# shaohua-pan/RobustCap

Measured on AMD Instinct MI355X. Metric: body-frames/sec (sig_mp fwd + FK) at batch 256, higher is better.
Workload: dtype f32; 1 GPU; synthetic 60 fps, 6 IMU + 33 keypoints, batch 256 x 1448 frames per GPU (256 bodies in total, weak scaling), confidence schedule 'mixed', seeded random weights (63.4 M params); batch_per_gpu=256, bodies_total=256, frames=1448, conf=mixed, parallelism=dp1 (sequence sharding)

## Files before the change

### include/robustcap_hip.h

```cpp
#ifndef ROBUSTCAP_HIP_H
#define ROBUSTCAP_HIP_H

#include <stdint.h>

#ifdef __cplusplus
extern "C" {
#endif

typedef struct rc_ctx rc_ctx;

typedef enum {
    RC_OK = 0,
    RC_ERR_INVALID = -1,
    RC_ERR_HIP = -2,
    RC_ERR_STATE = -3,
    RC_ERR_UNKNOWN_KEY = -4
} rc_status;

typedef struct {
    double conf_lo, conf_hi;
    float contact_threshold;
    float distance_threshold;
    float height_threshold;
    double tran_filter_num;
    int32_t use_flat_floor;
    int32_t use_vision_updater;
    int32_t use_imu_updater;
    int32_t live;
    int32_t update_vision_freq;
    int32_t use_reproj_opt;
    float smooth;
    int32_t reserved;
} rc_params;

#define RC_FLAG_FIRST_FRAME 1u

int rc_create(int32_t batch, int32_t live_at_construction, rc_ctx** out);
int rc_destroy(rc_ctx* ctx);
const char* rc_last_error(const rc_ctx* ctx);
int rc_default_params(int32_t live_at_construction, rc_params* out);
int rc_get_params(const rc_ctx* ctx, rc_params* out);
int rc_set_params(rc_ctx* ctx, const rc_params* p);

int rc_load_weight(rc_ctx* ctx, const char* key, const float* host, int64_t numel);
int rc_finalize_weights(rc_ctx* ctx);

int rc_set_body(rc_ctx* ctx, const int32_t* parent, const float* J, const float* w33, const float* v33);

int rc_set_gravity(rc_ctx* ctx, const float* gravity_host);

int rc_reset(rc_ctx* ctx, const uint8_t* row_mask, void* stream);

int rc_step(rc_ctx* ctx, const float* j2dc, const float* accc, const float* oric, const float* first_tran,
            uint32_t flags, float* pose_out, float* tran_out, void* stream);

int rc_sequence(rc_ctx* ctx, int32_t T, const float* j2dc, int64_t rs_j2d, const float* accc, int64_t rs_acc,
                const float* oric, int64_t rs_ori, const float* first_tran, uint32_t flags, float* pose_out,
                int64_t rs_pose, float* tran_out, int64_t rs_tran, void* stream);

int rc_sequence_rows(rc_ctx* ctx, int32_t T, const int32_t* len_host, const float* j2dc, int64_t rs_j2d, const float* accc,
                     int64_t rs_acc, const float* oric, int64_t rs_ori, const float* first_tran, uint32_t flags, float* pose_out,
                     int64_t rs_pose, float* tran_out, int64_t rs_tran, void* stream);
int rc_get_sequence_row_frames(rc_ctx* ctx, int64_t* body_frames);

int rc_set_gemm_mode(rc_ctx* ctx, int32_t mode);
int rc_get_gemm_mode(const rc_ctx* ctx);
int rc_default_gemm_mode(int32_t total_rows);

int rc_set_sequence_mode(rc_ctx* ctx, int32_t mode, int32_t min_frames);
int rc_get_sequence_stats(rc_ctx* ctx, int64_t* wave_frames, int64_t* stepped_frames, int64_t* ticks);
int rc_get_launch_stats(rc_ctx* ctx, int64_t* lds_launches, int64_t* other_wide_launches);
int rc_get_launch_stats_w32(rc_ctx* ctx, int64_t* w32_launches);
int rc_set_resident(rc_ctx* ctx, int32_t enable, int32_t workgroups);
int rc_get_resident_stats(rc_ctx* ctx, int64_t* segments, int64_t* aborts);
int rc_plan_sequence(const int8_t* codes, int32_t B, int32_t T, const int32_t* pend, uint32_t flags, int32_t use_vision_updater,
                     uint8_t* mode_out);
int rc_plan_wave(const int8_t* codes, int32_t B, int32_t T, int32_t t0, const int32_t* first_reach, const int32_t* pend,
                 int32_t use_imu_updater, int32_t use_vision_updater, int32_t* frame_at, int64_t frame_at_cap,
                 int32_t* n_ticks, int32_t* n_prep, int32_t* counts, double* est_us);
int rc_plan_wave_rows(const int8_t* codes, int32_t B, int32_t T, int32_t t0, const int32_t* len, const int32_t* first_reach,
                      const int32_t* pend, int32_t use_imu_updater, int32_t use_vision_updater, int32_t* frame_at, int64_t frame_at_cap,
                      int32_t* n_ticks, int32_t* n_prep, int32_t* counts, double* est_us);

int rc_live_begin(rc_ctx* ctx);
int rc_live_step(rc_ctx* ctx, const float* j2dc_host, const float* accc_host, const float* oric_host,
                 const float* first_tran_host, uint32_t flags, float* pose_host, float* tran_host);
int rc_live_end(rc_ctx* ctx);
int rc_get_live_stats(rc_ctx* ctx, int64_t* lean_frames, int64_t* full_frames);
int rc_get_live_prestep(rc_ctx* ctx, int64_t* presteps, int32_t* available);
int rc_get_live_replayed(rc_ctx* ctx, int64_t* frames);
int rc_get_live_spin(rc_ctx* ctx, int64_t* taken, int64_t* lost);
int rc_get_live_profile(rc_ctx* ctx, double* avg_us4);
int rc_get_live_last_profile(rc_ctx* ctx, double* us6);
int rc_get_live_backend(rc_ctx* ctx, int32_t* lean_captured, int32_t* aql, char* note, int32_t note_len);

int rc_r6d_to_rotmat(const float* r6d, float* R, int64_t n, void* stream);
int rc_axis_angle_to_rotmat(const float* aa, float* R, int64_t n, void* stream);
int rc_rotmat_to_axis_angle(const float* R, float* aa, int64_t n, void* stream);
int rc_rotmat_to_r6d(const float* R, float* r6d, int64_t n, void* stream);
int rc_angle_between(const float* R1, const float* R2, float* out, int64_t n, void* stream);
int rc_lerp(const float* a, const float* b, double t, float* out, int64_t n, void* stream);
int rc_normalize_rows(const float* x, float* out, float* norm, int64_t rows, int32_t width, void* stream);
int rc_bbox_normalise(const float* kp, float* out, int64_t n, void* stream);
int rc_conf_mean(const float* j2dc, int64_t n, double lo, double hi, float* mean, int8_t* code, void* stream);
int rc_shape_body(rc_ctx* ctx, const float* v_template, const float* shapedirs, const float* J_regressor, const float* beta,
                  int32_t V, float* verts_out, float* joints_out);
int rc_fk_r(rc_ctx* ctx, const float* Rlocal, float* Rglobal, int64_t n, void* stream);
int rc_bone_to_joint(rc_ctx* ctx, const float* bone, float* joint, int64_t n, void* stream);
int rc_joint_to_bone(rc_ctx* ctx, const float* joint, float* bone, int64_t n, void* stream);
int rc_zero_pose(rc_ctx* ctx, float* joint, float* vert, void* stream);
int rc_ik_r(rc_ctx* ctx, const float* Rglobal, float* Rlocal, int64_t n, void* stream);
int rc_fk_bone(rc_ctx* ctx, const float* Rglobal, float* joints, int64_t n, void* stream);
int rc_body_fk(rc_ctx* ctx, const float* pose, const float* tran, float* grot, float* joint, float* j33,
               int64_t n, void* stream);
int rc_lstm_step(rc_ctx* ctx, const char* net, const float* x, const uint8_t* row_mask, float* y, void* stream);
#define RC_SUBNET_SCRATCH_BYTES (256ll << 20)
int rc_subnet_forward(rc_ctx* ctx, const char* net, int32_t n, const int32_t* lengths_host, const float* x, float* y,
                      const float* init_h, const float* init_c, float* final_h, float* final_c, void* stream);
int rc_subnet_forward_tape(rc_ctx* ctx, const char* net, int32_t n, const int32_t* lengths_host, const float* x, float* y,
                           const float* init_h, const float* init_c, float* final_h, float* final_c, float* acts, float* tape,
                           void* stream);
int rc_subnet_tape_floats(rc_ctx* ctx, const char* net, int32_t n, const int32_t* lengths_host, int64_t* floats);
int rc_subnet_backward(rc_ctx* ctx, const char* net, int32_t n, const int32_t* lengths_host, const float* tape, const float* d_h1,
                       const float* d_final_h, const float* d_final_c, float* d_gates, float* d_a, float* d_init_h, float* d_init_c,
                       void* stream);
int rc_dropout_apply(rc_ctx* ctx, const float* src, float* dst, int64_t rows, int32_t cols, int32_t site, float p, uint64_t seed,
                     uint32_t call, void* stream);
int rc_subnet_forward_train(rc_ctx* ctx, const char* net, int32_t n, const int32_t* lengths_host, const float* x, float* y,
                            const float* init_h, const float* init_c, float* final_h, float* final_c, float* acts, float* tape, float p,
                            uint64_t seed, uint32_t call, void* stream);
int rc_subnet_backward_train(rc_ctx* ctx, const char* net, int32_t n, const int32_t* lengths_host, const float* tape, const float* d_h1,
                             const float* d_final_h, const float* d_final_c, float* d_gates, float* d_a, float* d_init_h,
                             float* d_init_c, float p, uint64_t seed, uint32_t call, void* stream);
int rc_update_subnet_weights(rc_ctx* ctx, const char* net, const void* const* tensors_dev, int32_t count, void* stream);
int rc_subnet_optim_step(rc_ctx* ctx, const char* net, const void* const* params_dev, const void* const* grads_dev,
                         const void* const* exp_avg_dev, const void* const* exp_avg_sq_dev, int32_t count, double lr, double beta1,
                         double beta2, double eps, double weight_decay, double bias_correction1, double bias_correction2, double max_norm,
                         float* norm_out_dev, void* stream);
int rc_init_net_forward(rc_ctx* ctx, int32_t n, const float* v, float* out, void* stream);
int rc_get_subnet_stats(rc_ctx* ctx, int64_t* calls, int64_t* frames, int64_t* chunks, int64_t* scratch_bytes);
int rc_set_mesh(rc_ctx* ctx, const float* v_template_host, const float* weights_host, int32_t V);
int rc_body_mesh(rc_ctx* ctx, const float* pose, const float* tran, float* vert, int64_t n, void* stream);
int rc_set_regressor(rc_ctx* ctx, const float* j_regressor_host, int32_t n_rows, int32_t n_used);
int rc_mesh_metrics(rc_ctx* ctx, const float* pose, const float* gt_pose, int64_t n, float* per_frame, double* mean_host,
                    void* stream);
int rc_synth_imu(rc_ctx* ctx, const float* pose, const float* tran, const int32_t* vertex_ids_host,
                 const int32_t* joint_ids_host, int64_t T, int32_t smooth_n, float* imu_ori, float* imu_acc, float* joint3d,
                 float* vert6, void* stream);
int rc_syn_acc(const float* v, int64_t T, int64_t width, int32_t smooth_n, float* acc, void* stream);
int rc_procrustes_error(const float* S1, const float* S2, int64_t n, int32_t n_points, float* err, void* stream);
int rc_position_error(const float* p, const float* t, int64_t n, float* dist, double* mean_host, void* stream);
int rc_set_ignored_landmarks(rc_ctx* ctx, const int32_t* ids_host, int32_t n);
int rc_reproj_residual(rc_ctx* ctx, const float* pose, const float* tran, const float* kp, const float* K,
                       float sigma, float* loss, int64_t T, void* stream);


int rc_smplify_set_prior(rc_ctx* ctx, const float* means_host, const float* precisions_host, const float* nll_weights_host);

int rc_smplify_loss_grad(rc_ctx* ctx, const float* x, const float* kp, const float* ref3d, const float* imu_aa,
                         const float* K_host, int64_t T, double* loss_host, float* grad, void* stream);

int rc_smplify_set_ref3d(rc_ctx* ctx, const float* ref3d);

typedef struct rc_smplify_info {
    int32_t status;
    int32_t n_iter, n_eval;
    int32_t reserved;
    double first_loss, final_loss;
    double host_ms, device_ms;
} rc_smplify_info;

int rc_smplify_run(rc_ctx* ctx, const float* pose, const float* tran, const float* kp, const float* imu_ori,
                   const float* K_host, int64_t T, float lr, int32_t max_iter, float loss_threshold, float* pose_out,
                   float* tran_out, uint8_t* update_host, rc_smplify_info* info, void* stream);

int rc_smplify_run_batch(rc_ctx* ctx, int32_t n_rows, const int64_t* T_rows, const float* const* pose, const float* const* tran,
                         const float* const* kp, const float* const* imu_ori, const float* K_host, float lr, int32_t max_iter,
                         float loss_threshold, float* const* pose_out, float* const* tran_out, uint8_t* const* update_host,
                         rc_smplify_info* infos, void* stream);

typedef double (*rc_objective_fn)(void* user, const double* x, double* grad, int64_t n);
int rc_lbfgs_minimize(rc_objective_fn objective, void* user, int64_t n, double* x, double lr, int32_t max_iter,
                      int32_t max_eval, int32_t history_size, double tolerance_grad, double tolerance_change,
                      int32_t* n_iter_out, int32_t* n_eval_out, double* losses_out, int64_t cap);

int rc_camera_inputs(const float* kp_pix, const float* imu_acc_w, const float* imu_ori_w, const float* K_host,
                     const float* Tcw_host, float* j2dc, float* accc, float* oric, float* gravity_out_host, int64_t n,
                     void* stream);

int rc_camera_inputs_rows(const float* kp_norm, const float* imu_acc_w, const float* imu_ori_w, const int32_t* seq_of_row,
                          const int32_t* len, const float* K_host, const float* Tcw_host, float image_w, float image_h,
                          int32_t n_rows, int32_t Tmax, float* j2dc, float* accc, float* oric, float* gravity_out_host,
                          void* cam_scratch, void* stream);

int rc_get_state(rc_ctx* ctx, const char* net, float* h_host, float* c_host, void* stream);
int rc_get_fusion_state(rc_ctx* ctx, int32_t* out_host, void* stream);

int rc_get_trace(rc_ctx* ctx, int32_t* trace_host, void* stream);

int rc_gemm_timing(rc_ctx* ctx, int32_t enable);
int rc_gemm_timing_read(rc_ctx* ctx, double* total_ms, int64_t* launches);
int rc_gemm_timing_busy(rc_ctx* ctx, double* busy_ms);

#ifdef __cplusplus
}
#endif
#endif
```

### robustcap_amd/_lib.py

```python
import ctypes as C
import os

_HERE = os.path.dirname(os.path.abspath(__file__))
LIB_PATH = os.environ.get("RC_LIB_PATH") or os.path.join(_HERE, "csrc", "librobustcap_hip.so")
HEADER_PATH = os.path.join(os.path.dirname(_HERE), "include", "robustcap_hip.h")

RC_FLAG_FIRST_FRAME = 1


class RcParams(C.Structure):
    _fields_ = [("conf_lo", C.c_double), ("conf_hi", C.c_double),
                ("contact_threshold", C.c_float), ("distance_threshold", C.c_float),
                ("height_threshold", C.c_float), ("tran_filter_num", C.c_double),
                ("use_flat_floor", C.c_int32), ("use_vision_updater", C.c_int32),
                ("use_imu_updater", C.c_int32), ("live", C.c_int32),
                ("update_vision_freq", C.c_int32), ("use_reproj_opt", C.c_int32), ("smooth", C.c_float),
                ("reserved", C.c_int32)]


class RcSmplifyInfo(C.Structure):
    _fields_ = [("status", C.c_int32), ("n_iter", C.c_int32), ("n_eval", C.c_int32), ("reserved", C.c_int32),
                ("first_loss", C.c_double), ("final_loss", C.c_double), ("host_ms", C.c_double), ("device_ms", C.c_double)]


OBJECTIVE_FN = C.CFUNCTYPE(C.c_double, C.c_void_p, C.POINTER(C.c_double), C.POINTER(C.c_double), C.c_int64)


class RobustcapLibraryError(RuntimeError):
    pass


_P, _I32, _I64, _U32, _F = C.c_void_p, C.c_int32, C.c_int64, C.c_uint32, C.c_float
SIGNATURES = {
    "rc_create": (_I32, [_I32, _I32, C.POINTER(_P)]),
    "rc_destroy": (_I32, [_P]),
    "rc_last_error": (C.c_char_p, [_P]),
    "rc_default_params": (_I32, [_I32, C.POINTER(RcParams)]),
    "rc_get_params": (_I32, [_P, C.POINTER(RcParams)]),
    "rc_set_params": (_I32, [_P, C.POINTER(RcParams)]),
    "rc_load_weight": (_I32, [_P, C.c_char_p, _P, _I64]),
    "rc_finalize_weights": (_I32, [_P]),
    "rc_set_body": (_I32, [_P, _P, _P, _P, _P]),
    "rc_set_gravity": (_I32, [_P, _P]),
    "rc_reset": (_I32, [_P, _P, _P]),
    "rc_step": (_I32, [_P, _P, _P, _P, _P, _U32, _P, _P, _P]),
    "rc_sequence": (_I32, [_P, _I32, _P, _I64, _P, _I64, _P, _I64, _P, _U32, _P, _I64, _P, _I64, _P]),
    "rc_sequence_rows": (_I32, [_P, _I32, _P, _P, _I64, _P, _I64, _P, _I64, _P, _U32, _P, _I64, _P, _I64, _P]),
    "rc_get_sequence_row_frames": (_I32, [_P, C.POINTER(_I64)]),
    "rc_set_gemm_mode": (_I32, [_P, _I32]),
    "rc_get_gemm_mode": (_I32, [_P]),
    "rc_default_gemm_mode": (_I32, [_I32]),
    "rc_set_sequence_mode": (_I32, [_P, _I32, _I32]),
    "rc_get_sequence_stats": (_I32, [_P, C.POINTER(_I64), C.POINTER(_I64), C.POINTER(_I64)]),
    "rc_get_launch_stats": (_I32, [_P, C.POINTER(_I64), C.POINTER(_I64)]),
    "rc_get_launch_stats_w32": (_I32, [_P, C.POINTER(_I64)]),
    "rc_set_resident": (_I32, [_P, _I32, _I32]),
    "rc_get_resident_stats": (_I32, [_P, C.POINTER(_I64), C.POINTER(_I64)]),
    "rc_plan_sequence": (_I32, [_P, _I32, _I32, _P, _U32, _I32, _P]),
    "rc_plan_wave": (_I32, [_P, _I32, _I32, _I32, _P, _P, _I32, _I32, _P, _I64, C.POINTER(_I32), C.POINTER(_I32), _P, _P]),
    "rc_plan_wave_rows": (_I32, [_P, _I32, _I32, _I32, _P, _P, _P, _I32, _I32, _P, _I64, C.POINTER(_I32), C.POINTER(_I32), _P, _P]),
    "rc_live_begin": (_I32, [_P]),
    "rc_live_step": (_I32, [_P, _P, _P, _P, _P, _U32, _P, _P]),
    "rc_live_end": (_I32, [_P]),
    "rc_get_live_stats": (_I32, [_P, _P, _P]),
    "rc_get_live_prestep": (_I32, [_P, _P, _P]),
    "rc_get_live_replayed": (_I32, [_P, _P]),
    "rc_get_live_spin": (_I32, [_P, _P, _P]),
    "rc_get_live_profile": (_I32, [_P, _P]),
    "rc_get_live_last_profile": (_I32, [_P, _P]),
    "rc_get_live_backend": (_I32, [_P, _P, _P, _P, _I32]),
    "rc_get_fusion_state": (_I32, [_P, _P, _P]),
    "rc_r6d_to_rotmat": (_I32, [_P, _P, _I64, _P]),
    "rc_axis_angle_to_rotmat": (_I32, [_P, _P, _I64, _P]),
    "rc_rotmat_to_axis_angle": (_I32, [_P, _P, _I64, _P]),
    "rc_rotmat_to_r6d": (_I32, [_P, _P, _I64, _P]),
    "rc_angle_between": (_I32, [_P, _P, _P, _I64, _P]),
    "rc_lerp": (_I32, [_P, _P, C.c_double, _P, _I64, _P]),
    "rc_normalize_rows": (_I32, [_P, _P, _P, _I64, _I32, _P]),
    "rc_bbox_normalise": (_I32, [_P, _P, _I64, _P]),
    "rc_conf_mean": (_I32, [_P, _I64, C.c_double, C.c_double, _P, _P, _P]),
    "rc_shape_body": (_I32, [_P, _P, _P, _P, _P, _I32, _P, _P]),
    "rc_fk_r": (_I32, [_P, _P, _P, _I64, _P]),
    "rc_bone_to_joint": (_I32, [_P, _P, _P, _I64, _P]),
    "rc_joint_to_bone": (_I32, [_P, _P, _P, _I64, _P]),
    "rc_zero_pose": (_I32, [_P, _P, _P, _P]),
    "rc_ik_r": (_I32, [_P, _P, _P, _I64, _P]),
    "rc_fk_bone": (_I32, [_P, _P, _P, _I64, _P]),
    "rc_body_fk": (_I32, [_P, _P, _P, _P, _P, _P, _I64, _P]),
    "rc_set_mesh": (_I32, [_P, _P, _P, _I32]),
    "rc_body_mesh": (_I32, [_P, _P, _P, _P, _I64, _P]),
    "rc_set_regressor": (_I32, [_P, _P, _I32, _I32]),
    "rc_mesh_metrics": (_I32, [_P, _P, _P, _I64, _P, C.POINTER(C.c_double), _P]),
    "rc_synth_imu": (_I32, [_P, _P, _P, _P, _P, _I64, _I32, _P, _P, _P, _P, _P]),
    "rc_syn_acc": (_I32, [_P, _I64, _I64, _I32, _P, _P]),
    "rc_procrustes_error": (_I32, [_P, _P, _I64, _I32, _P, _P]),
    "rc_position_error": (_I32, [_P, _P, _I64, _P, C.POINTER(C.c_double), _P]),
    "rc_lstm_step": (_I32, [_P, C.c_char_p, _P, _P, _P, _P]),
    "rc_subnet_forward": (_I32, [_P, C.c_char_p, _I32, _P, _P, _P, _P, _P, _P, _P, _P]),
    "rc_subnet_forward_tape": (_I32, [_P, C.c_char_p, _I32, _P, _P, _P, _P, _P, _P, _P, _P, _P, _P]),
    "rc_subnet_tape_floats": (_I32, [_P, C.c_char_p, _I32, _P, C.POINTER(_I64)]),
    "rc_subnet_backward": (_I32, [_P, C.c_char_p, _I32, _P, _P, _P, _P, _P, _P, _P, _P, _P, _P]),
    "rc_dropout_apply": (_I32, [_P, _P, _P, _I64, _I32, _I32, _F, C.c_uint64, _U32, _P]),
    "rc_subnet_forward_train": (_I32, [_P, C.c_char_p, _I32, _P, _P, _P, _P, _P, _P, _P, _P, _P, _F, C.c_uint64, _U32, _P]),
    "rc_subnet_backward_train": (_I32, [_P, C.c_char_p, _I32, _P, _P, _P, _P, _P, _P, _P, _P, _P, _F, C.c_uint64, _U32, _P]),
    "rc_update_subnet_weights": (_I32, [_P, C.c_char_p, _P, _I32, _P]),
    "rc_subnet_optim_step": (_I32, [_P, C.c_char_p, _P, _P, _P, _P, _I32] + [C.c_double] * 8 + [_P, _P]),
    "rc_init_net_forward": (_I32, [_P, _I32, _P, _P, _P]),
    "rc_get_subnet_stats": (_I32, [_P, C.POINTER(_I64), C.POINTER(_I64), C.POINTER(_I64), C.POINTER(_I64)]),
    "rc_set_ignored_landmarks": (_I32, [_P, _P, _I32]),
    "rc_reproj_residual": (_I32, [_P, _P, _P, _P, _P, _F, _P, _I64, _P]),
    "rc_smplify_set_prior": (_I32, [_P, _P, _P, _P]),
    "rc_smplify_set_ref3d": (_I32, [_P, _P]),
    "rc_smplify_loss_grad": (_I32, [_P, _P, _P, _P, _P, _P, _I64, C.POINTER(C.c_double), _P, _P]),
    "rc_smplify_run": (_I32, [_P, _P, _P, _P, _P, _P, _I64, _F, _I32, _F, _P, _P, _P, C.POINTER(RcSmplifyInfo), _P]),
    "rc_smplify_run_batch": (_I32, [_P, _I32, _P, _P, _P, _P, _P, _P, _F, _I32, _F, _P, _P, _P, _P, _P]),
    "rc_lbfgs_minimize": (_I32, [OBJECTIVE_FN, _P, _I64, C.POINTER(C.c_double), C.c_double, _I32, _I32, _I32, C.c_double,
                                 C.c_double, C.POINTER(_I32), C.POINTER(_I32), C.POINTER(C.c_double), _I64]),
    "rc_camera_inputs": (_I32, [_P, _P, _P, _P, _P, _P, _P, _P, _P, _I64, _P]),
    "rc_camera_inputs_rows": (_I32, [_P, _P, _P, _P, _P, _P, _P, _F, _F, _I32, _I32, _P, _P, _P, _P, _P, _P]),
    "rc_get_state": (_I32, [_P, C.c_char_p, _P, _P, _P]),
    "rc_get_trace": (_I32, [_P, _P, _P]),
    "rc_gemm_timing": (_I32, [_P, _I32]),
    "rc_gemm_timing_read": (_I32, [_P, C.POINTER(C.c_double), C.POINTER(_I64)]),
    "rc_gemm_timing_busy": (_I32, [_P, C.POINTER(C.c_double)]),
}

_lib = None


OPTIONAL_IN_AB_BUILDS = frozenset({"rc_get_launch_stats_w32", "rc_set_resident", "rc_get_resident_stats", "rc_get_launch_stats", "rc_get_live_spin", "rc_get_live_replayed", "rc_get_live_profile", "rc_get_live_last_profile",
                                   "rc_get_live_prestep"})


def load():
    global _lib
    if _lib is not None:
        return _lib
    if not os.path.exists(LIB_PATH):
        raise RobustcapLibraryError(
            f"{LIB_PATH} not found: the HIP extension is not built. Run "
            "`python -c \"import __graft_entry__ as g; g.build()\"` at the repo root. There is no CPU fallback.")
    try:
        lib = C.CDLL(LIB_PATH)
    except OSError as e:
        raise RobustcapLibraryError(f"cannot load {LIB_PATH}: {e}") from e
    ab_build = bool(os.environ.get("RC_LIB_PATH"))
    skipped = []
    for name, (res, args) in SIGNATURES.items():
        if ab_build and name in OPTIONAL_IN_AB_BUILDS and not hasattr(lib, name):
            skipped.append(name)
            continue
        try:
            fn = getattr(lib, name)
        except AttributeError as e:
            raise RobustcapLibraryError(f"{LIB_PATH} does not export {name}: the library does not match include/robustcap_hip.h") from e
        fn.restype, fn.argtypes = res, args
    if skipped:
        import warnings
        warnings.warn(f"RC_LIB_PATH={LIB_PATH}: entry points missing in this build (calls to them will fail): {', '.join(skipped)}")
    _lib = lib
    return lib


def check(ctx, rc, what):
    if rc != 0:
        msg = load().rc_last_error(ctx)
        raise RobustcapLibraryError(f"{what} failed ({rc}): {msg.decode() if msg else ''}")


def ptr(t):
    return None if t is None else C.c_void_p(t.data_ptr())


def stream_ptr():
    import torch
    return C.c_void_p(torch.cuda.current_stream().cuda_stream)
```

### robustcap_amd/csrc/rc_api.cpp

```cpp
#include "../../include/robustcap_hip.h"
#include "rc_ctx.h"

#include <algorithm>
#include <cmath>
#include <cstdio>
#include <cstdlib>
#include <cstring>
#include <map>
#include <string>
#include <thread>
#include <vector>

static thread_local std::string g_create_error;

int fail(rc_ctx* ctx, int code, const std::string& msg) {
    if (ctx) ctx->err = msg; else g_create_error = msg;
    return code;
}

namespace {

const int kInit[3][2] = {{69, 512}, {512, 1024}, {1024, 2048}};

template <typename Body>
// ... 385 lines not shown
    if (!ctx) return RC_ERR_INVALID;
    if (!net || !tensors_dev) return fail(ctx, RC_ERR_INVALID, "rc_update_subnet_weights: null argument");
    const int ni = net_index(net);
    if (ni < 0) return fail(ctx, RC_ERR_INVALID, std::string("rc_update_subnet_weights: unknown net ") + net);
    const int want = ni == N2 ? 18 : 12;
    if (count != want) return fail(ctx, RC_ERR_INVALID, "rc_update_subnet_weights: " + std::string(net) + " has " + std::to_string(want) + " tensors");
    for (int i = 0; i < count; ++i)
        if (!tensors_dev[i]) return fail(ctx, RC_ERR_INVALID, "rc_update_subnet_weights: null tensor");
    if (!ctx->have_weights) return fail(ctx, RC_ERR_STATE, "rc_update_subnet_weights: weights not finalized");
    hipStream_t st = (hipStream_t)stream;
    auto T = [&](int i) { return static_cast<const float*>(tensors_dev[i]); };
    live_forget_last_frame(ctx);
    if (int rc = live_discard_ahead(ctx)) return rc;
    HIP_TRY(ctx, hipDeviceSynchronize());
    NetDev& n = ctx->net[ni];
    auto dense = [&](Dense& d, const float* W, const float* b) -> int {
        rc_launch_repack_dense(W, d.N, d.K, d.Np, d.Kp, d.W, d.Ws, st);
        if (d.Wrm) HIP_TRY(ctx, hipMemcpyAsync(d.Wrm, W, (size_t)d.N * d.K * sizeof(float), hipMemcpyDeviceToDevice, st));
        HIP_TRY(ctx, hipMemcpyAsync(d.b, b, (size_t)d.N * sizeof(float), hipMemcpyDeviceToDevice, st));
        return RC_OK;
    };
    for (int l = 0; l < 2; ++l) rc_launch_repack_lstm(T(4 * l), T(4 * l + 1), T(4 * l + 2), T(4 * l + 3), n.H, n.Wl[l], n.Wls[l], n.bl[l], st);
    if (int rc = dense(n.lin1, T(8), T(9))) return rc;
    if (int rc = dense(n.lin2, T(10), T(11))) return rc;
    if (ni == N2)
        for (int q = 0; q < 3; ++q)
            if (int rc = dense(ctx->init[q], T(12 + 2 * q), T(13 + 2 * q))) return rc;
    rc_subnet_retranspose(ctx->subnet.get(), ni, n.Wl, n.H, ctx->weights_epoch, st);
    HIP_TRY(ctx, hipGetLastError());
    HIP_TRY(ctx, hipStreamSynchronize(st));
    return RC_OK;
}

static long long subnet_tensor_numel(int ni, int i) {
    const NetSpec& s = kNets[ni];
    const long long H = s.H;
    if (i < 8) return (i & 3) < 2 ? 4 * H * H : 4 * H;
    if (i < 12) return i == 8 ? H * s.in : i == 9 ? H : i == 10 ? (long long)s.out * H : s.out;
    const int q = (i - 12) / 2;
    return (i & 1) ? kInit[q][1] : (long long)kInit[q][0] * kInit[q][1];
}

int rc_subnet_optim_step(rc_ctx* ctx, const char* net, const void* const* params_dev, const void* const* grads_dev,
                         const void* const* exp_avg_dev, const void* const* exp_avg_sq_dev, int32_t count, double lr, double beta1,
                         double beta2, double eps, double weight_decay, double bias_correction1, double bias_correction2, double max_norm,
                         float* norm_out_dev, void* stream) {
    if (!ctx) return RC_ERR_INVALID;
    const char* what = "rc_subnet_optim_step: ";
    if (!net || !params_dev || !grads_dev || !exp_avg_dev || !exp_avg_sq_dev || !norm_out_dev)
        return fail(ctx, RC_ERR_INVALID, std::string(what) + "null argument");
    const int ni = net_index(net);
    if (ni < 0) return fail(ctx, RC_ERR_INVALID, std::string(what) + "unknown net " + net);
    const int want = ni == N2 ? 18 : 12;
    if (count != want) return fail(ctx, RC_ERR_INVALID, what + std::string(net) + " has " + std::to_string(want) + " tensors");
    for (int i = 0; i < count; ++i)
        if (!params_dev[i] || !exp_avg_dev[i] || !exp_avg_sq_dev[i]) return fail(ctx, RC_ERR_INVALID, std::string(what) + "null parameter or moment tensor");
    if (!(bias_correction1 > 0.0) || !(bias_correction2 > 0.0)) return fail(ctx, RC_ERR_INVALID, std::string(what) + "bias corrections must be positive");
    if (!ctx->have_weights) return fail(ctx, RC_ERR_STATE, std::string(what) + "weights not finalized");
    hipStream_t st = (hipStream_t)stream;
    if (!ctx->optim_partial) {
        long long most = 0;
        for (int j = 0; j < 6; ++j) {
            long long b = 0;
            for (int i = 0; i < (j == N2 ? 18 : 12); ++i) b += (subnet_tensor_numel(j, i) + RC_OPTIM_CHUNK - 1) / RC_OPTIM_CHUNK;
            most = std::max(most, b);
        }
        HIP_TRY(ctx, rc_alloc(ctx->optim_partial, (size_t)most));
    }
    OptimNorm nrm{};
    nrm.count = count;
    int blocks = 0;
    for (int i = 0; i < count; ++i) {
        nrm.g[i] = static_cast<const float*>(grads_dev[i]);
        nrm.n[i] = subnet_tensor_numel(ni, i);
        nrm.block0[i] = blocks;
        if (nrm.g[i]) blocks += (int)((nrm.n[i] + RC_OPTIM_CHUNK - 1) / RC_OPTIM_CHUNK);
    }
    nrm.block0[count] = blocks;
    OptimScalars a{};
    a.step_size = (float)(lr / bias_correction1); a.bc2_sqrt = (float)std::sqrt(bias_correction2);
    a.beta1 = (float)beta1; a.one_m_beta1 = (float)(1.0 - beta1); a.beta2 = (float)beta2; a.one_m_beta2 = (float)(1.0 - beta2);
    a.eps = (float)eps; a.weight_decay = (float)weight_decay;
    auto T = [&](int i) {
        return OptimTensor{static_cast<float*>(const_cast<void*>(params_dev[i])), static_cast<const float*>(grads_dev[i]),
                           static_cast<float*>(const_cast<void*>(exp_avg_dev[i])), static_cast<float*>(const_cast<void*>(exp_avg_sq_dev[i]))};
    };
    for (int i : {0, 1, 4, 5}) {
        const OptimTensor t = T(i);
        if (((uintptr_t)t.p | (uintptr_t)t.g | (uintptr_t)t.m | (uintptr_t)t.v) & 15)
            return fail(ctx, RC_ERR_INVALID, std::string(what) + "the LSTM weight tensors must be 16-byte aligned");
    }
    live_forget_last_frame(ctx);
    const bool live = live_session_open(ctx);
    if (live) {
        if (int rc = live_discard_ahead(ctx)) return rc;
        HIP_TRY(ctx, hipDeviceSynchronize());
    }
    rc_launch_optim_norm(nrm, blocks, ctx->optim_partial.get(), (float)max_norm, norm_out_dev, st);
    NetDev& n = ctx->net[ni];
    auto dense = [&](Dense& d, int i) { rc_launch_optim_dense(T(i), T(i + 1), d.N, d.K, d.Np, d.Kp, d.W, d.Ws, d.Wrm, d.b, a, norm_out_dev, st); };
    for (int l = 0; l < 2; ++l)
        rc_launch_optim_lstm(T(4 * l), T(4 * l + 1), T(4 * l + 2), T(4 * l + 3), n.H, n.Wl[l], n.Wls[l], n.bl[l], a, norm_out_dev, st);
    dense(n.lin1, 8);
    dense(n.lin2, 10);
    if (ni == N2)
        for (int q = 0; q < 3; ++q) dense(ctx->init[q], 12 + 2 * q);
    rc_subnet_retranspose(ctx->subnet.get(), ni, n.Wl, n.H, ctx->weights_epoch, st);
    HIP_TRY(ctx, hipGetLastError());
    if (live) {
        HIP_TRY(ctx, hipStreamSynchronize(st));
        return RC_OK;
    }
    return mark_eager(ctx, st);
}

static int finalize_weights_impl(rc_ctx* ctx) {
    for (int i = 0; i < 6; ++i) {
        const NetSpec& s = kNets[i];
        NetDev& n = ctx->net[i];
        const std::string p = std::string(s.name) + ".";
        const size_t H = s.H;
        auto need = [&](const std::string& r, size_t numel) { return staged(ctx, p + r, numel); };
        const auto *w1 = need("linear1.weight", H * s.in), *b1 = need("linear1.bias", H);
        const auto *w2 = need("linear2.weight", (size_t)s.out * H), *b2 = need("linear2.bias", s.out);
        if (!w1 || !b1 || !w2 || !b2) return fail(ctx, RC_ERR_STATE, "rc_finalize_weights: missing linear weights of " + p);
        if (int rc = make_dense(ctx, n.lin1, *w1, *b1, s.H, s.in)) return rc;
        if (int rc = make_dense(ctx, n.lin2, *w2, *b2, s.out, s.H)) return rc;
        for (int l = 0; l < 2; ++l) {
            const std::string sl = std::to_string(l);
            const auto *wi = need("rnn.weight_ih_l" + sl, 4 * H * H), *wh = need("rnn.weight_hh_l" + sl, 4 * H * H);
            const auto *bi = need("rnn.bias_ih_l" + sl, 4 * H), *bh = need("rnn.bias_hh_l" + sl, 4 * H);
            if (!wi || !wh || !bi || !bh) return fail(ctx, RC_ERR_STATE, "rc_finalize_weights: missing LSTM weights of " + p);
            auto orig = [&](int np) { const int cb = np / 16, u = (np % 16) / 4, g = np % 4; return (size_t)g * H + 4 * cb + u; };
            auto get = [&](int np, int k) -> float {
                const size_t r = orig(np);
                return k < (int)H ? (*wi)[r * H + k] : (*wh)[r * H + (k - H)];
            };
            std::vector<float> bp(4 * H);
            for (size_t np = 0; np < 4 * H; ++np) bp[np] = (*bi)[orig((int)np)] + (*bh)[orig((int)np)];
            if (int rc = upload(ctx, &n.Wl[l], pack_weights(4 * s.H, 2 * s.H, get))) return rc;
            if (int rc = upload16(ctx, &n.Wls[l], pack_weights_split(4 * s.H, 2 * s.H, get))) return rc;
            if (int rc = upload(ctx, &n.bl[l], bp)) return rc;
        }
    }
    for (int q = 0; q < 3; ++q) {
        const std::string p = "rnn2.init_net." + std::to_string(2 * q) + ".";
        const auto *w = staged(ctx, p + "weight", (size_t)kInit[q][0] * kInit[q][1]), *b = staged(ctx, p + "bias", kInit[q][1]);
        if (!w || !b) return fail(ctx, RC_ERR_STATE, "rc_finalize_weights: missing " + p);
        if (int rc = make_dense(ctx, ctx->init[q], *w, *b, kInit[q][1], kInit[q][0])) return rc;
    }
    ctx->have_weights = true;
    const bool aw = ctx->alloc_weights;
    ctx->alloc_weights = false;
    const int rc_pre = seq_prepare(ctx);
    ctx->alloc_weights = aw;
    if (rc_pre) return rc_pre;
    HIP_TRY(ctx, hipDeviceSynchronize());
    std::map<std::string, std::vector<float>>().swap(ctx->staged);
    return RC_OK;
}

int rc_set_body(rc_ctx* ctx, const int32_t* parent, const float* J, const float* w33, const float* v33) {
    if (!ctx || !parent || !J || !w33 || !v33) return RC_ERR_INVALID;
    BodyConst b{};
    for (int i = 0; i < 24; ++i) {
        b.parent[i] = i == 0 ? 0 : parent[i];
        if (i > 0 && (parent[i] < 0 || parent[i] >= i)) return fail(ctx, RC_ERR_INVALID, "rc_set_body: parent[i] must be in [0, i)");
        b.level[i] = i == 0 ? 0 : b.level[parent[i]] + 1;
        if (b.level[i] > 9) return fail(ctx, RC_ERR_INVALID, "rc_set_body: kinematic tree deeper than 9");
        if (i > 0) {
            int& n = b.nchild[parent[i]];
            if (n >= 4) return fail(ctx, RC_ERR_INVALID, "rc_set_body: a joint with more than 4 children");
            b.child[parent[i]][n++] = i;
        }
    }
    for (int i = 0; i < 24; ++i)
        for (int c = 0; c < 3; ++c) {
            b.jroot[c] = J[c];
            b.jrest[i][c] = J[3 * i + c] - J[c];
            b.bone[i][c] = i == 0 ? b.jrest[0][c] : (J[3 * i + c] - J[c]) - (J[3 * parent[i] + c] - J[c]);
        }
    for (int v = 0; v < 33; ++v) {
        b.override_joint[v] = -1;
        for (int c = 0; c < 3; ++c) b.v33[v][c] = v33[3 * v + c] - J[c];
        for (int j = 0; j < 24; ++j) b.w33[v][j] = w33[24 * v + j];
    }
    const int ov[12][2] = {{11, 16}, {12, 17}, {13, 18}, {14, 19}, {15, 20}, {16, 21},
                           {23, 1},  {24, 2},  {25, 4},  {26, 5},  {27, 7},  {28, 8}};
    for (auto& o : ov) b.override_joint[o[0]] = o[1];
    HIP_TRY(ctx, hipMemcpy(ctx->body, &b, sizeof(b), hipMemcpyHostToDevice));
    ctx->have_body = true;
    for (int c = 0; c < 3; ++c) ctx->jroot_h[c] = b.jroot[c];
    ctx->fold_dirty = true;
    return RC_OK;
}

int rc_set_gravity(rc_ctx* ctx, const float* g) {
    if (!ctx || !g) return RC_ERR_INVALID;
    HIP_TRY(ctx, hipMemcpy(ctx->fb.gravity, g, (size_t)ctx->B * 3 * sizeof(float), hipMemcpyHostToDevice));
    return RC_OK;
}

int rc_reset(rc_ctx* ctx, const uint8_t* row_mask, void* stream) {
    if (!ctx) return RC_ERR_INVALID;
    live_forget_last_frame(ctx, true);
    float* h[6]; float* c[6]; int H[6];
    for (int i = 0; i < 6; ++i) { h[i] = ctx->net[i].h; c[i] = ctx->net[i].c; H[i] = ctx->net[i].H; }
    rc_launch_reset(ctx->fb, h, c, H, row_mask, ctx->B, (hipStream_t)stream);
    HIP_TRY(ctx, hipGetLastError());
    return mark_eager(ctx, (hipStream_t)stream);
}

int rc_step(rc_ctx* ctx, const float* j2dc, const float* accc, const float* oric, const float* first_tran, uint32_t flags,
            float* pose_out, float* tran_out, void* stream) {
    if (int rc = check_ready(ctx)) return rc;
    live_forget_last_frame(ctx);
    if (!j2dc || !accc || !oric || !pose_out || !tran_out) return fail(ctx, RC_ERR_INVALID, "rc_step: null buffer");
    FrameIO io{j2dc, accc, oric, first_tran, pose_out, tran_out, 99, 18, 54, 216, 3};
    if (int rc = step_impl(ctx, io, flags, (hipStream_t)stream)) return rc;
    return mark_eager(ctx, (hipStream_t)stream);
}

int rc_r6d_to_rotmat(const float* r6d, float* R, int64_t n, void* stream) {
    if (n == 0) return RC_OK;
    if (!r6d || !R || n < 0) return RC_ERR_INVALID;
    rc_launch_r6d(r6d, R, n, (hipStream_t)stream);
    return hipGetLastError() == hipSuccess ? RC_OK : RC_ERR_HIP;
}
int rc_axis_angle_to_rotmat(const float* aa, float* R, int64_t n, void* stream) {
    if (n == 0) return RC_OK;
    if (!aa || !R || n < 0) return RC_ERR_INVALID;
    rc_launch_aa2R(aa, R, n, (hipStream_t)stream);
    return hipGetLastError() == hipSuccess ? RC_OK : RC_ERR_HIP;
}
int rc_rotmat_to_axis_angle(const float* R, float* aa, int64_t n, void* stream) {
    if (n == 0) return RC_OK;
    if (!aa || !R || n < 0) return RC_ERR_INVALID;
    rc_launch_R2aa(R, aa, n, (hipStream_t)stream);
    return hipGetLastError() == hipSuccess ? RC_OK : RC_ERR_HIP;
}
int rc_rotmat_to_r6d(const float* R, float* r6d, int64_t n, void* stream) {
    if (n == 0) return RC_OK;
    if (!R || !r6d || n < 0) return RC_ERR_INVALID;
    rc_launch_rotmat_to_r6d(R, r6d, n, (hipStream_t)stream);
    return hipGetLastError() == hipSuccess ? RC_OK : RC_ERR_HIP;
}
int rc_angle_between(const float* R1, const float* R2, float* out, int64_t n, void* stream) {
    if (n == 0) return RC_OK;
    if (!R1 || !R2 || !out || n < 0) return RC_ERR_INVALID;
    rc_launch_angle_between(R1, R2, out, n, (hipStream_t)stream);
    return hipGetLastError() == hipSuccess ? RC_OK : RC_ERR_HIP;
}
int rc_lerp(const float* a, const float* b, double t, float* out, int64_t n, void* stream) {
    if (n == 0) return RC_OK;
    if (!a || !b || !out || n < 0) return RC_ERR_INVALID;
    rc_launch_lerp(a, b, (float)(1.0 - t), (float)t, out, n, (hipStream_t)stream);
    return hipGetLastError() == hipSuccess ? RC_OK : RC_ERR_HIP;
}
int rc_normalize_rows(const float* x, float* out, float* norm, int64_t rows, int32_t width, void* stream) {
    if (rows == 0) return RC_OK;
    if (!x || !out || rows < 0 || width < 1) return RC_ERR_INVALID;
    rc_launch_normalize_rows(x, out, norm, rows, width, (hipStream_t)stream);
    return hipGetLastError() == hipSuccess ? RC_OK : RC_ERR_HIP;
}
int rc_bbox_normalise(const float* kp, float* out, int64_t n, void* stream) {
    if (n == 0) return RC_OK;
    if (!kp || !out || n < 0) return RC_ERR_INVALID;
    rc_launch_bbox_normalise(kp, out, n, (hipStream_t)stream);
    return hipGetLastError() == hipSuccess ? RC_OK : RC_ERR_HIP;
}
int rc_conf_mean(const float* j2dc, int64_t n, double lo, double hi, float* mean, int8_t* code, void* stream) {
    if (n == 0) return RC_OK;
    if (!j2dc || (!mean && !code) || n < 0 || n > INT32_MAX) return RC_ERR_INVALID;
    rc_launch_scan_conf(j2dc, 99, (int)n, 1, lo, hi, (signed char*)code, (hipStream_t)stream, mean);
    return hipGetLastError() == hipSuccess ? RC_OK : RC_ERR_HIP;
}
int rc_fk_r(rc_ctx* ctx, const float* Rl, float* Rg, int64_t n, void* stream) {
    if (!ctx || !ctx->have_body) return ctx ? fail(ctx, RC_ERR_STATE, "rc_fk_r: body not set") : RC_ERR_INVALID;
    if (n < 0 || (n > 0 && (!Rl || !Rg))) return fail(ctx, RC_ERR_INVALID, "rc_fk_r: bad argument");
    rc_launch_fk_r(ctx->body, Rl, Rg, n, (hipStream_t)stream);
    HIP_TRY(ctx, hipGetLastError());
    return RC_OK;
}
int rc_bone_to_joint(rc_ctx* ctx, const float* bone, float* joint, int64_t n, void* stream) {
    if (!ctx || !ctx->have_body) return ctx ? fail(ctx, RC_ERR_STATE, "rc_bone_to_joint: body not set") : RC_ERR_INVALID;
    if (n < 0 || (n > 0 && (!bone || !joint))) return fail(ctx, RC_ERR_INVALID, "rc_bone_to_joint: bad argument");
    rc_launch_bone_to_joint(ctx->body, bone, joint, n, (hipStream_t)stream);
    HIP_TRY(ctx, hipGetLastError());
    return RC_OK;
}
int rc_joint_to_bone(rc_ctx* ctx, const float* joint, float* bone, int64_t n, void* stream) {
    if (!ctx || !ctx->have_body) return ctx ? fail(ctx, RC_ERR_STATE, "rc_joint_to_bone: body not set") : RC_ERR_INVALID;
    if (n < 0 || (n > 0 && (!bone || !joint))) return fail(ctx, RC_ERR_INVALID, "rc_joint_to_bone: bad argument");
    rc_launch_joint_to_bone(ctx->body, joint, bone, n, (hipStream_t)stream);
    HIP_TRY(ctx, hipGetLastError());
    return RC_OK;
}
int rc_zero_pose(rc_ctx* ctx, float* joint, float* vert, void* stream) {
    if (!ctx || !ctx->have_body) return ctx ? fail(ctx, RC_ERR_STATE, "rc_zero_pose: body not set") : RC_ERR_INVALID;
    if (!joint) return fail(ctx, RC_ERR_INVALID, "rc_zero_pose: null buffer");
    if (vert && ctx->mesh_V == 0) return fail(ctx, RC_ERR_STATE, "rc_zero_pose: vertices need rc_set_mesh");
    rc_launch_zero_pose(ctx->body, ctx->mesh_vt, ctx->mesh_V, joint, vert, (hipStream_t)stream);
    HIP_TRY(ctx, hipGetLastError());
    return RC_OK;
}
int rc_shape_body(rc_ctx* ctx, const float* v_template, const float* shapedirs, const float* J_regressor, const float* beta,
                  int32_t V, float* verts_out, float* joints_out) {
// ... 280 lines not shown
```

### robustcap_amd/csrc/rc_ctx.h

```cpp
#pragma once
#include "../../include/robustcap_hip.h"
#include "rc_internal.h"

#include <map>
#include <string>
#include <type_traits>
#include <utility>
#include <vector>

struct NetSpec { const char* name; int in, H, out; };
const NetSpec kNets[6] = {{"rnn2", 72, 512, 69},  {"rnn3", 141, 512, 3},   {"rnn4", 171, 1280, 69},
                          {"rnn6", 240, 1024, 3}, {"rnn7", 141, 512, 144}, {"rnn8", 141, 512, 2}};
enum { N2 = 0, N3 = 1, N4 = 2, N6 = 3, N7 = 4, N8 = 5 };

inline int round_up(int x, int m) { return (x + m - 1) / m * m; }

struct Dense {
    float* W = nullptr; float* b = nullptr;
    void* Ws = nullptr;
    float* Wrm = nullptr;
    int K = 0, N = 0, Kp = 0, Np = 0;
    int mr = 2, nc = 4;
};
struct NetDev {
    Dense lin1, lin2;
    float* Wl[2] = {nullptr, nullptr};
    void* Wls[2] = {nullptr, nullptr};
    float* bl[2] = {nullptr, nullptr};
    float* h = nullptr;
    float* c = nullptr;
    int* steps = nullptr;
    float* x1 = nullptr;
    float* part = nullptr;
    int in = 0, H = 0, out = 0;
    int nc = 4;
    int mr = 2;
};

struct rc_ctx {
    int B = 0;
    int Bp = 0;
    int dev = 0;
    rc_params prm{};
    NetDev net[6];
    Dense init[3];
    float *hid1 = nullptr, *hid2 = nullptr, *xtmp = nullptr;
    FrameBuffers fb{};
    BodyConst* body = nullptr;
    float *mesh_vt = nullptr, *mesh_w = nullptr;
    int mesh_V = 0;
    float* mesh_kM = nullptr;
    int mesh_nk = 0;
    std::vector<float> mesh_vt_h, mesh_w_h, mesh_Jr_h;
    float jroot_h[3] = {0.f, 0.f, 0.f};
    bool fold_dirty = false;
    DevBuf<float> sweep_scratch;
    size_t sweep_scratch_cap = 0;
    unsigned long long ign_mask = RC_IGN_DEFAULT;
    bool have_body = false, have_weights = false;
    long long weights_epoch = 0;
    std::map<std::string, std::vector<float>> staged;
    std::vector<DevBuf<char>> allocs;
    std::vector<std::pair<void*, size_t>> alloc_bytes;
    std::vector<DevBuf<char>> weight_allocs;
    bool alloc_weights = false;
    std::string err;
    LiveOwner live;
    SeqOwner seq;
    GemmOwner gemm;
    SmplifyOwner smplify;
    SubnetOwner subnet;
    DevBuf<double> optim_partial;
};

#pragma GCC visibility push(hidden)
int fail(rc_ctx* ctx, int code, const std::string& msg);
int tune_env(const char* name, int dflt);
int check_ready(rc_ctx* ctx);
rc_params_dev dev_params(const rc_params& p);
int step_impl(rc_ctx* ctx, const FrameIO& io, uint32_t flags, hipStream_t st, bool with_tr = true, bool skip_prep = false,
              const FrameIO* next_io = nullptr, int n_live = -1);
template <typename T>
int dev_alloc(rc_ctx* ctx, T** p, size_t count, bool zero = true) {
    DevBuf<char> q;
    HIP_TRY(ctx, rc_alloc(q, count * sizeof(T)));
    if (zero) HIP_TRY(ctx, hipMemset(q.get(), 0, count * sizeof(T)));
    *p = reinterpret_cast<T*>(q.get());
    if (!ctx->alloc_weights) ctx->alloc_bytes.emplace_back(q.get(), count * sizeof(T));
    (ctx->alloc_weights ? ctx->weight_allocs : ctx->allocs).push_back(std::move(q));
    return RC_OK;
}
int gemm_create(rc_ctx* ctx);
struct Out { float* p; int ld; int col0; bool packed; };
struct Stage {
    int net; int flag_bit; const float* x; int ldx; Out y;
    const unsigned char* flags = nullptr;
    const float* x_alt = nullptr;
    int sel_bit = 0;
    int out_bit = 0;
    int rows_hint = -1;
};
GemmSeg seg(const float* base, int ld, int K, int mode = RC_PAR_NONE, long long stride = 0);
GemmProblem dense_problem(const rc_ctx* ctx, const Dense& d, GemmSeg a, Out out, bool relu, int flag_bit, const unsigned char* flags, int* steps,
                          bool open_step);
GemmProblem lin1_problem(const rc_ctx* c, const Stage& s);
GemmProblem lstm_problem(const rc_ctx* c, const Stage& s, int layer);
GemmProblem lin2_problem(const rc_ctx* c, const Stage& s);
bool tile_env(const char* name, int* mr, int* nc);
void pick_tile(int H, int rows, int* mr, int* nc);
bool gemm_split(const rc_ctx* c);
bool lds_context(const rc_ctx* c);
bool lds_problem(const rc_ctx* c, int rows);
struct LdsRegion { float* slab; int* tickets; size_t tiles; };
int lds_region(rc_ctx* ctx, size_t r, LdsRegion* out);
int build_lds_problems(rc_ctx* ctx, const std::vector<GemmProblem>& ps, const unsigned char* flags_override, float* slab, int* tickets,
                       LdsProblem* out, int max_p, int* items, size_t* tiles_out, bool resident_order = false);
int launch_problems(rc_ctx* ctx, std::vector<GemmProblem> ps, const unsigned char* flags_override, hipStream_t st, bool fp32 = false,
                    hipEvent_t stop = nullptr, bool* launched = nullptr);
enum LaunchKind { LAUNCH_SHARED, LAUNCH_WIDE, LAUNCH_SMALL, LAUNCH_RESIDENT };
int timed_launch_impl(rc_ctx* ctx, hipStream_t st, LaunchKind kind, void (*issue)(void*), void* arg);
template <class F> int timed_launch(rc_ctx* ctx, hipStream_t st, LaunchKind kind, F&& issue) {
    return timed_launch_impl(ctx, st, kind, [](void* f) { (*static_cast<std::remove_reference_t<F>*>(f))(); }, &issue);
}
bool resident_launch_fits_timing(const rc_ctx* c);
void count_resident_launch(rc_ctx* ctx);
struct LiveLaunchScope { rc_ctx* ctx; explicit LiveLaunchScope(rc_ctx* c); ~LiveLaunchScope(); };
struct TimingSuspended { rc_ctx* ctx; bool was; explicit TimingSuspended(rc_ctx* c); ~TimingSuspended(); };
void seq_create(rc_ctx* ctx);
int seq_prepare(rc_ctx* ctx);
void seq_weights_changed(rc_ctx* ctx);
bool seq_is_engine_stream(const rc_ctx* ctx, hipStream_t st);
void live_create(rc_ctx* ctx);
void live_forget_last_frame(rc_ctx* ctx, bool rows_reset = false);
int live_discard_ahead(rc_ctx* ctx);
int mark_eager(rc_ctx* ctx, hipStream_t st);
bool live_session_open(const rc_ctx* ctx);
#pragma GCC visibility pop
```

### robustcap_amd/csrc/rc_gemm_api.cpp

```cpp
#include "../../include/robustcap_hip.h"
#include "rc_ctx.h"

#include <algorithm>
#include <cstdio>
#include <cstdlib>
#include <cstring>
#include <string>
#include <vector>

#define RC_SPLIT_MIN_BATCH 48
#define RC_TILE64_MIN_BATCH 192

#ifndef RC_NC1280
#define RC_NC1280 10
#endif

const int kLdsRegions = 12;

#pragma GCC visibility push(hidden)

struct GemmLauncher {
    bool split = false;
    bool live_launch = false;
    unsigned live_nt_mask = 63u;
    int tile4[2] = {4, 5}, tile6[2] = {4, 8}, tile378[2] = {4, 4}, tile2[2] = {0, 0};
    int trace_next = 0;
    bool timing = false;
    int timing_mode = 1;
    std::vector<std::pair<HipEvent, HipEvent>> ev_pool;
    size_t ev_used = 0;
    double timed_ms = 0.0;
    double timed_busy_ms = 0.0;
    long long timed_launches = 0;
    long long stat_wide_launches = 0;
    long long stat_lds_launches = 0;
    long long stat_w32_launches = 0;
    int lds_min_rows = 64;
    int lds_min_batch = 65;
    int lds_ksplit[3] = {1, 2, 2};
    bool lds_block_pick = true;
    DevBuf<float> lds_slab;
    DevBuf<int> lds_tickets;
    size_t lds_region_tiles = 0;
    unsigned lds_rot = 0;
};

void rc_gemm_free(GemmLauncher* g) { delete g; }

static int default_gemm_mode(int rows) { return tune_env("RC_GEMM_SPLIT", rows >= RC_SPLIT_MIN_BATCH ? 1 : 0) != 0 ? 1 : 0; }

int gemm_create(rc_ctx* ctx) {
    ctx->gemm.reset(new GemmLauncher());
    GemmLauncher& g = *ctx->gemm;
    const int batch = ctx->B;
    g.split = default_gemm_mode(batch) != 0;
    g.live_nt_mask = (unsigned)tune_env("RC_LIVE_NT_MASK", 63);
    g.lds_min_rows = tune_env("RC_LDS_MIN_ROWS", std::min(160, std::max(64, batch / 2)));
    g.lds_min_batch = tune_env("RC_LDS_MIN_BATCH", g.lds_min_batch);
    g.lds_block_pick = tune_env("RC_LDS_BLOCK_PICK", 1) != 0;
    g.lds_ksplit[0] = tune_env("RC_LDS_KSPLIT_512", 1) == 1 ? 1 : 2;
    g.lds_ksplit[1] = tune_env("RC_LDS_KSPLIT_1024", batch <= 160 ? 1 : 2) == 1 ? 1 : 2;
    g.lds_ksplit[2] = tune_env("RC_LDS_KSPLIT_1280", 2) == 1 ? 1 : 2;
    const struct { const char* knob; int* tile; int H; } tiles[4] = {{"RC_TILE_RNN6", g.tile6, 1024}, {"RC_TILE_S2H512", g.tile378, 512},
                                                                     {"RC_TILE_RNN2", g.tile2, 512}, {"RC_TILE_RNN4", g.tile4, 1280}};
    for (const auto& t : tiles) tile_env(t.knob, &t.tile[0], &t.tile[1]);
    for (const auto& t : tiles)
        if (t.tile[1] > 0 && t.H % (4 * t.tile[1]) != 0)
            return fail(nullptr, RC_ERR_INVALID, std::string("rc_create: ") + t.knob + " tile width of " + std::to_string(4 * t.tile[1]) +
                                                 " units does not divide H = " + std::to_string(t.H));
    return RC_OK;
}

bool gemm_split(const rc_ctx* c) { return c->gemm->split; }
bool lds_context(const rc_ctx* c) { return c->gemm->split && c->gemm->lds_min_rows > 0 && c->B >= c->gemm->lds_min_batch; }
bool lds_problem(const rc_ctx* c, int rows) { return lds_context(c) && rows >= c->gemm->lds_min_rows; }

LiveLaunchScope::LiveLaunchScope(rc_ctx* c) : ctx(c) { ctx->gemm->live_launch = true; }
LiveLaunchScope::~LiveLaunchScope() { ctx->gemm->live_launch = false; }
TimingSuspended::TimingSuspended(rc_ctx* c) : ctx(c), was(c->gemm->timing) { ctx->gemm->timing = false; }
TimingSuspended::~TimingSuspended() { ctx->gemm->timing = was; }

GemmSeg seg(const float* base, int ld, int K, int mode, long long stride) {
    GemmSeg s{};
    s.base = base; s.ld = ld; s.K = K; s.par_mode = mode; s.par_stride = stride;
    return s;
}

GemmProblem dense_problem(const rc_ctx* ctx, const Dense& d, GemmSeg a, Out out, bool relu, int flag_bit,
                          const unsigned char* flags, int* steps, bool open_step) {
    GemmProblem p{};
    a.K = d.Kp;
    p.seg[0] = a;
    p.seg[1] = seg(a.base, a.ld, 0);
    p.W = d.W; p.Ws = d.Ws; p.bias = d.b; p.out = out.p; p.ldo = out.ld; p.N = d.N; p.out_col0 = out.col0; p.out_packed = out.packed ? 1 : 0;
    p.steps = steps; p.flags = flags; p.flag_bit = flag_bit;
    p.epi = relu ? RC_EPI_RELU : RC_EPI_DENSE;
    p.open_step = open_step ? 1 : 0;
    const bool narrow = ctx->B <= 16 || d.N <= 160;
    const int mr = narrow ? 1 : d.mr, nc = narrow ? 1 : d.nc;
    p.n_tiles = nc == 1 ? (d.N + 15) / 16 : d.Np / (16 * nc);
    p.m_tiles = (ctx->B + 16 * mr - 1) / (16 * mr); p.Kp = d.Kp; p.nc = nc; p.mr = mr;
    return p;
}

bool tile_env(const char* name, int* mr, int* nc) {
    const char* v = std::getenv(name);
    int a = 0, b = 0;
    if (!v || std::sscanf(v, "%dx%d", &a, &b) != 2) return false;
    const int code = a * 16 + b;
    for (int ok : {2 * 16 + 4, 4 * 16 + 4, 8 * 16 + 4, 2 * 16 + 8, 4 * 16 + 8, 2 * 16 + 10, 4 * 16 + 5})
        if (code == ok) { *mr = a; *nc = b; return true; }
    return false;
}

void pick_tile(int H, int rows, int* mr, int* nc) {
    if (rows >= 128) { *mr = 2; *nc = H == 1280 ? RC_NC1280 : (H == 1024 ? 8 : 4); return; }
    if (rows > 16) { *mr = 2; *nc = rows >= 64 ? 4 : 2; if (*nc == 2) { *mr = 1; } return; }
    *mr = 1; *nc = 1;
}

GemmProblem lin1_problem(const rc_ctx* c, const Stage& s) {
    const NetDev& n = c->net[s.net];
    GemmProblem p = dense_problem(c, n.lin1, seg(s.x, s.ldx, 0), Out{n.x1, n.H, 0, true}, true, s.flag_bit,
                                  s.flags ? s.flags : c->fb.flags, n.steps, true);
    if (s.rows_hint >= 0 && s.rows_hint <= 16) {
        p.mr = 1; p.nc = 1; p.n_tiles = (n.lin1.N + 15) / 16;
    }
    if (s.rows_hint >= 0 && s.rows_hint < c->B) p.m_tiles = (s.rows_hint + 16 * p.mr - 1) / (16 * p.mr);
    p.alt_base = s.x_alt; p.sel_flags = c->fb.flags; p.sel_bit = s.x_alt ? s.sel_bit : 0;
    p.nt = (c->gemm->live_nt_mask >> s.net) & 1u;
    return p;
}
GemmProblem lstm_problem(const rc_ctx* c, const Stage& s, int layer) {
    const GemmLauncher& g = *c->gemm;
    const NetDev& n = c->net[s.net];
    const long long BH = (long long)c->Bp * n.H;
    GemmProblem p{};
    if (layer == 0) p.seg[0] = seg(n.x1, n.H, n.H);
    else p.seg[0] = seg(n.h, n.H, n.H, RC_PAR_DST, BH);
    p.seg[1] = seg(n.h + layer * RC_HBUF * BH, n.H, n.H, RC_PAR_SRC, BH);
    p.W = n.Wl[layer]; p.Ws = n.Wls[layer]; p.bias = n.bl[layer];
    p.hstate = n.h + layer * RC_HBUF * BH; p.cstate = n.c + layer * (long long)c->B * n.H; p.h_par_stride = BH; p.H = n.H;
    p.steps = n.steps; p.flags = s.flags ? s.flags : c->fb.flags; p.flag_bit = s.flag_bit;
    p.epi = RC_EPI_LSTM;
    int mr, nc;
    pick_tile(n.H, s.rows_hint < 0 ? c->B : s.rows_hint, &mr, &nc);
    if (s.rows_hint < 0 && c->B >= RC_TILE64_MIN_BATCH) {
        if (s.net == N6 && g.tile6[0]) { mr = g.tile6[0]; nc = g.tile6[1]; }
        if ((s.net == N3 || s.net == N7 || s.net == N8) && g.tile378[0]) { mr = g.tile378[0]; nc = g.tile378[1]; }
        if (s.net == N2 && g.tile2[0]) { mr = g.tile2[0]; nc = g.tile2[1]; }
        if (s.net == N4 && g.tile4[0]) { mr = g.tile4[0]; nc = g.tile4[1]; }
    }
    const int rows = s.rows_hint < 0 ? c->B : (s.rows_hint < c->B ? s.rows_hint : c->B);
    if (lds_problem(c, rows)) { mr = 16; nc = 8; }
    p.n_tiles = n.H / (4 * nc); p.m_tiles = (rows + 16 * mr - 1) / (16 * mr); p.Kp = 2 * n.H; p.nc = nc; p.mr = mr;
    p.nt = (g.live_nt_mask >> s.net) & 1u;
    return p;
}
GemmProblem lin2_problem(const rc_ctx* c, const Stage& s) {
    const NetDev& n = c->net[s.net];
    const long long BH = (long long)c->Bp * n.H;
    GemmProblem p = dense_problem(c, n.lin2, seg(n.h + RC_HBUF * BH, n.H, 0, RC_PAR_DST, BH), s.y, false, s.flag_bit,
                                  s.flags ? s.flags : c->fb.flags, n.steps, false);
    p.out_flags = c->fb.flags; p.out_bit = s.out_bit;
    p.nt = 1;
    return p;
}

static int ensure_lds_pool(rc_ctx* ctx) {
    GemmLauncher& g = *ctx->gemm;
    if (g.lds_slab) return RC_OK;
    const size_t m_tiles = ((size_t)ctx->B + 255) / 256;
    const size_t tiles = 320 * m_tiles;
    HIP_TRY(ctx, rc_alloc(g.lds_slab, (size_t)kLdsRegions * tiles * RC_LDS_SLAB_FLOATS));
    HIP_TRY(ctx, rc_alloc(g.lds_tickets, (size_t)kLdsRegions * tiles));
    HIP_TRY(ctx, hipMemset(g.lds_tickets.get(), 0, (size_t)kLdsRegions * tiles * sizeof(int)));
    g.lds_region_tiles = tiles;
    return RC_OK;
}

int lds_region(rc_ctx* ctx, size_t r, LdsRegion* out) {
    if (int rc = ensure_lds_pool(ctx)) return rc;
    const GemmLauncher& g = *ctx->gemm;
    out->slab = g.lds_slab.get() + r * g.lds_region_tiles * RC_LDS_SLAB_FLOATS;
    out->tickets = g.lds_tickets.get() + r * g.lds_region_tiles;
    out->tiles = g.lds_region_tiles;
    return RC_OK;
}

static bool timing_pair(GemmLauncher& g, hipEvent_t* a, hipEvent_t* b) {
    if (g.ev_used == g.ev_pool.size()) {
        std::pair<HipEvent, HipEvent> ev;
        if (hipEventCreate(rc_out(ev.first)) != hipSuccess || hipEventCreate(rc_out(ev.second)) != hipSuccess) return false;
        g.ev_pool.push_back(std::move(ev));
    }
    const auto& ev = g.ev_pool[g.ev_used++];
    *a = ev.first.get(); *b = ev.second.get();
    return true;
}

static bool is_timed(const GemmLauncher& g, LaunchKind kind) {
    if (!g.timing) return false;
    if (g.timing_mode == 3) return kind == LAUNCH_SHARED || kind == LAUNCH_RESIDENT;
    return !(g.timing_mode == 2 && kind == LAUNCH_SMALL);
}
bool resident_launch_fits_timing(const rc_ctx* c) { return !(c->gemm->timing && c->gemm->timing_mode != 3); }
void count_resident_launch(rc_ctx* ctx) { ctx->gemm->stat_lds_launches += 1; }

int timed_launch_impl(rc_ctx* ctx, hipStream_t st, LaunchKind kind, void (*issue)(void*), void* arg) {
    hipEvent_t a = nullptr, b = nullptr;
    if (is_timed(*ctx->gemm, kind) && !timing_pair(*ctx->gemm, &a, &b)) return fail(ctx, RC_ERR_HIP, "hipEventCreate");
    if (a) HIP_TRY(ctx, hipEventRecord(a, st));
    issue(arg);
    if (b) HIP_TRY(ctx, hipEventRecord(b, st));
    return RC_OK;
}

int build_lds_problems(rc_ctx* ctx, const std::vector<GemmProblem>& ps, const unsigned char* flags_override, float* slab, int* tickets,
                       LdsProblem* out, int max_p, int* items, size_t* tiles_out, bool resident_order) {
    std::vector<GemmProblem> ord(ps);
    auto key = [&](const GemmProblem& g) -> int {
        if (g.epi == RC_EPI_LSTM) return (resident_order && g.H == 512) ? 0 : g.Kp;
        return 1;
    };
    std::stable_sort(ord.begin(), ord.end(), [&](const GemmProblem& a, const GemmProblem& b) { return key(a) > key(b); });
    if ((int)ord.size() > max_p) return 0;
    int base = 0;
    size_t tiles = 0;
    for (size_t i = 0; i < ord.size(); ++i) {
        const GemmProblem& g = ord[i];
        LdsProblem& p = out[i];
        p = LdsProblem{};
        p.seg[0] = g.seg[0]; p.seg[1] = g.seg[1];
        p.Ws = g.Ws; p.bias = g.bias; p.hstate = g.hstate; p.cstate = g.cstate; p.steps = g.steps;
        p.flags = flags_override ? flags_override : g.flags; p.flag_bit = g.flag_bit;
        p.h_par_stride = g.h_par_stride; p.H = g.H; p.step_off = g.step_off;
        p.m_tiles = g.m_tiles; p.Qs = g.Kp / 32;
        p.epi = g.epi;
        p.block_pick = ctx->gemm->lds_block_pick && ctx->B <= 256 && g.m_tiles == 1 ? 1 : 0;
        if (g.epi == RC_EPI_LSTM) {
            p.n_tiles = g.H / 32;
            p.ksplit = ctx->gemm->lds_ksplit[g.H == 512 ? 0 : (g.H == 1024 ? 1 : 2)];
        } else {
            const long long half = (long long)(g.Kp / 32) * 256;
            p.seg[0].K = g.Kp / 2;
            p.seg[1] = p.seg[0]; p.seg[1].base = g.seg[0].base + half;
            p.alt[0] = g.alt_base; p.alt[1] = g.alt_base ? g.alt_base + half : nullptr;
            p.sel_flags = g.sel_flags; p.sel_bit = g.alt_base ? g.sel_bit : 0;
            p.out = g.out; p.ldo = g.ldo;
            p.n_tiles = g.N / 128;
            p.ksplit = 1;
        }
        p.wg_base = base;
        p.slab = slab + tiles * RC_LDS_SLAB_FLOATS; p.tickets = tickets + tiles;
        tiles += (size_t)p.n_tiles * p.m_tiles;
        base += round_up(p.n_tiles * p.m_tiles * p.ksplit, 8);
    }
    *items = base; *tiles_out = tiles;
    return (int)ord.size();
}
static void build_lds_launch(rc_ctx* ctx, const std::vector<GemmProblem>& ps, const unsigned char* flags_override, const LdsRegion& region,
                             LdsLaunch& L, int* items, size_t* tiles_out) {
    L = LdsLaunch{};
    L.B = ctx->B;
    L.n = build_lds_problems(ctx, ps, flags_override, region.slab, region.tickets, L.p, RC_LDS_MAXP, items, tiles_out);
}

static int launch_lds(rc_ctx* ctx, const std::vector<GemmProblem>& ps_in, const unsigned char* flags_override, hipStream_t st, hipEvent_t stop, bool* launched) {
    static const int replicate = std::getenv("RC_DBG_REPLICATE") ? std::atoi(std::getenv("RC_DBG_REPLICATE")) : 1;
    std::vector<GemmProblem> ps(ps_in);
    for (int r = 1; r < replicate && (int)ps.size() + (int)ps_in.size() <= RC_LDS_MAXP; ++r) ps.insert(ps.end(), ps_in.begin(), ps_in.end());
    LdsRegion region{};
    if (int rc = lds_region(ctx, ctx->gemm->lds_rot % kLdsRegions, &region)) return rc;
    ctx->gemm->lds_rot += 1;
    LdsLaunch L{};
    int base = 0;
    size_t tiles = 0;
    build_lds_launch(ctx, ps, flags_override, region, L, &base, &tiles);
    if (tiles > region.tiles) return fail(ctx, RC_ERR_INVALID, "shared-weight launch: more tiles than its slab region holds");
    ctx->gemm->stat_lds_launches += 1;
    if (int rc = timed_launch(ctx, st, LAUNCH_SHARED, [&] { rc_launch_gemm_lds(L, base, st, stop); })) return rc;
    if (launched && stop) *launched = true;
    HIP_TRY(ctx, hipGetLastError());
    return RC_OK;
}

static int lay_out_launch(const rc_ctx* ctx, const std::vector<GemmProblem>& ps, const unsigned char* flags_override, bool split, GemmLaunch& L) {
    L = GemmLaunch{};
    L.B = ctx->B;
    L.split = split ? 1 : 0;
    L.live = ctx->gemm->live_launch ? 1 : 0;
    if ((int)ps.size() > RC_MAX_PROB) return -1;
    int base = 0;
    for (int unaligned = 0; unaligned < 2; ++unaligned)
        for (const GemmProblem& q : ps) {
            if (((q.n_tiles & 7) != 0) != (unaligned != 0)) continue;
            GemmProblem& p = L.p[L.n++];
            p = q;
            p.wg_base = base;
            if (flags_override) p.flags = flags_override;
            base += round_up(p.n_tiles * p.m_tiles, 8);
            p.trace_base = ctx->gemm->trace_next;
        }
    return base;
}

static bool dense_items_selftest_wanted(rc_ctx* ctx, const std::vector<GemmProblem>& ps, hipStream_t st, bool fp32) {
    static const int on = std::getenv("RC_DBG_DENSE_ITEMS") ? std::atoi(std::getenv("RC_DBG_DENSE_ITEMS")) : 0;
    if (!on || !ctx->gemm->split || fp32 || ctx->B > 256 || seq_is_engine_stream(ctx, st) || (int)ps.size() > RC_RES_MAXP) return false;
    for (const GemmProblem& p : ps)
        if (!(p.epi == RC_EPI_RELU && p.out_packed && p.N % 128 == 0 && p.Kp % 128 == 0 && p.out_bit == 0 && p.out_col0 == 0 && p.seg[0].par_mode == 0)) return false;
    return true;
}
static int dense_items_selftest(rc_ctx* ctx, const std::vector<GemmProblem>& ps, const unsigned char* flags_override, hipStream_t st) {
    LdsRegion region{};
    if (int rc = lds_region(ctx, 0, &region)) return rc;
    const int n_ints = 2 + RC_RES_MAXP + 1 + 4;
    DevBuf<ResidentTick> tk_d;
    DevBuf<int> ints_d;
    HIP_TRY(ctx, rc_alloc_all(tk_d, 1, ints_d, n_ints));
    ResidentTick T{};
    std::vector<GemmProblem> q(ps);
    for (GemmProblem& p : q) p.m_tiles = 1;
    size_t tiles = 0;
    T.B = ctx->B;
    T.n = build_lds_problems(ctx, q, flags_override, region.slab, region.tickets, T.p, RC_RES_MAXP, &T.n_items, &tiles, true);
    for (int i = 0; i < RC_RES_MAXP; ++i) T.dep[i][0] = T.dep[i][1] = -1;
    const int base[2] = {0, T.n_items};
    const size_t Bp = (size_t)ctx->Bp;
    HIP_TRY(ctx, hipStreamSynchronize(st));
    for (const GemmProblem& p : ps) HIP_TRY(ctx, hipMemset(p.out, 0xff, Bp * p.N * sizeof(float)));
    HIP_TRY(ctx, hipMemcpy(tk_d.get(), &T, sizeof(T), hipMemcpyHostToDevice));
    HIP_TRY(ctx, hipMemset(ints_d.get(), 0, n_ints * sizeof(int)));
    HIP_TRY(ctx, hipMemcpy(ints_d.get(), base, sizeof(base), hipMemcpyHostToDevice));
    ResidentArgs R{};
    R.ticks = tk_d.get(); R.item_base = ints_d.get(); R.n_ticks = 1;
    R.done = ints_d.get() + 2; R.tick_done = ints_d.get() + 2 + RC_RES_MAXP; R.head = ints_d.get() + 3 + RC_RES_MAXP; R.flag_tail = R.head + 1; R.abort = R.head + 2;
    R.spin_bound = 100000ull * 100;
    rc_launch_gemm_resident(R, 64, st);
    HIP_TRY(ctx, hipStreamSynchronize(st));
    std::vector<std::vector<float>> got(ps.size());
    for (size_t i = 0; i < ps.size(); ++i) {
        got[i].resize(Bp * ps[i].N);
        HIP_TRY(ctx, hipMemcpy(got[i].data(), ps[i].out, got[i].size() * sizeof(float), hipMemcpyDeviceToHost));
        HIP_TRY(ctx, hipMemset(ps[i].out, 0xff, got[i].size() * sizeof(float)));
    }
    {
        GemmLaunch L{};
        const int wg = lay_out_launch(ctx, ps, flags_override, true, L);
        if (wg < 0) return fail(ctx, RC_ERR_INVALID, "too many fused problems");
        rc_launch_gemm(L, wg, st, nullptr);
        HIP_TRY(ctx, hipStreamSynchronize(st));
    }
    for (size_t i = 0; i < ps.size(); ++i) {
        std::vector<float> ref(got[i].size());
        HIP_TRY(ctx, hipMemcpy(ref.data(), ps[i].out, ref.size() * sizeof(float), hipMemcpyDeviceToHost));
        size_t bad = 0, written = 0;
        for (size_t e = 0; e < ref.size(); ++e) {
            uint32_t r, g;
            std::memcpy(&r, &ref[e], 4); std::memcpy(&g, &got[i][e], 4);
            if (r == 0xffffffffu && g == 0xffffffffu) continue;
            ++written;
            if (r != g) ++bad;
        }
        std::fprintf(stderr, "[dbg dense] N %d Kp %d alt %d: %zu of %zu written elements differ\n", ps[i].N, ps[i].Kp, ps[i].alt_base ? 1 : 0, bad, written);
    }
    return RC_OK;
}

int launch_problems(rc_ctx* ctx, std::vector<GemmProblem> ps, const unsigned char* flags_override, hipStream_t st, bool fp32, hipEvent_t stop,
                    bool* launched) {
    GemmLauncher& g = *ctx->gemm;
    if (launched) *launched = false;
    if (ps.empty()) return RC_OK;
    if (dense_items_selftest_wanted(ctx, ps, st, fp32)) return dense_items_selftest(ctx, ps, flags_override, st);
    {
        std::vector<GemmProblem> lds, rest;
        for (GemmProblem& p : ps) {
            if (p.mr == 16) {
                if (g.split && !fp32 && p.epi == RC_EPI_LSTM && (int)lds.size() < RC_LDS_MAXP) { lds.push_back(p); continue; }
                p.mr = 4; p.nc = 8; p.m_tiles *= 4;
            }
            rest.push_back(p);
        }
        if (!lds.empty()) {
            if (!rest.empty()) if (int rc = launch_problems(ctx, rest, flags_override, st, fp32)) return rc;
            return launch_lds(ctx, lds, flags_override, st, stop, launched);
        }
    }
    if ((int)ps.size() > RC_MAX_PROB) {
        std::vector<GemmProblem> head(ps.begin(), ps.begin() + RC_MAX_PROB), tail(ps.begin() + RC_MAX_PROB, ps.end());
        if (int rc = launch_problems(ctx, head, flags_override, st, fp32)) return rc;
        return launch_problems(ctx, tail, flags_override, st, fp32, stop, launched);
    }
    GemmLaunch L{};
    const int base = lay_out_launch(ctx, ps, flags_override, g.split && !fp32, L);
    if (base < 0) return fail(ctx, RC_ERR_INVALID, "too many fused problems");
    g.trace_next = (g.trace_next + base) & 0x3fffffff;
    const bool small = rc_gemm_is_small(L);
    if (!small) g.stat_wide_launches += 1;
    if (rc_gemm_is_w32(L)) g.stat_w32_launches += 1;
    if (int rc = timed_launch(ctx, st, small ? LAUNCH_SMALL : LAUNCH_WIDE, [&] { rc_launch_gemm(L, base, st, stop); })) return rc;
    if (launched && stop) *launched = true;
    HIP_TRY(ctx, hipGetLastError());
    return RC_OK;
}

#pragma GCC visibility pop

int rc_ctx_gemm_split(rc_ctx* ctx) { return ctx->gemm->split ? 1 : 0; }

extern "C" {

int rc_set_gemm_mode(rc_ctx* ctx, int32_t mode) {
    if (!ctx || mode < 0 || mode > 1) return ctx ? fail(ctx, RC_ERR_INVALID, "rc_set_gemm_mode: 0 (fp32 MFMA) or 1 (split-bf16 products)") : RC_ERR_INVALID;
    if ((mode != 0) != ctx->gemm->split) rc_live_end(ctx);
    ctx->gemm->split = mode != 0;
    return RC_OK;
}
int rc_get_gemm_mode(const rc_ctx* ctx) { return ctx ? (ctx->gemm->split ? 1 : 0) : RC_ERR_INVALID; }
int rc_default_gemm_mode(int32_t total_rows) { return default_gemm_mode(total_rows); }

int rc_get_launch_stats_w32(rc_ctx* ctx, int64_t* w32_launches) {
    if (!ctx || !w32_launches) return RC_ERR_INVALID;
    *w32_launches = ctx->gemm->stat_w32_launches;
    return RC_OK;
}

int rc_get_launch_stats(rc_ctx* ctx, int64_t* tick_launches, int64_t* other_wide_launches) {
    if (!ctx) return RC_ERR_INVALID;
    if (tick_launches) *tick_launches = ctx->gemm->stat_lds_launches;
    if (other_wide_launches) *other_wide_launches = ctx->gemm->stat_wide_launches;
    return RC_OK;
}

int rc_gemm_timing(rc_ctx* ctx, int32_t enable) {
    if (!ctx) return RC_ERR_INVALID;
    GemmLauncher& g = *ctx->gemm;
    g.timing = enable != 0;
    if (enable) g.timing_mode = enable == 2 ? 2 : (enable == 3 ? 3 : 1);
    if (enable) { g.ev_used = 0; g.timed_ms = 0.0; g.timed_launches = 0; g.timed_busy_ms = 0.0; }
    return RC_OK;
}
int rc_gemm_timing_read(rc_ctx* ctx, double* total_ms, int64_t* launches) {
    if (!ctx || !total_ms || !launches) return RC_ERR_INVALID;
    GemmLauncher& g = *ctx->gemm;
    std::vector<std::pair<double, double>> iv;
    iv.reserve(g.ev_used);
    for (size_t i = 0; i < g.ev_used; ++i) {
        HIP_TRY(ctx, hipEventSynchronize(g.ev_pool[i].second.get()));
        float ms = 0.f, t0 = 0.f;
        HIP_TRY(ctx, hipEventElapsedTime(&ms, g.ev_pool[i].first.get(), g.ev_pool[i].second.get()));
        if (i > 0) HIP_TRY(ctx, hipEventElapsedTime(&t0, g.ev_pool[0].first.get(), g.ev_pool[i].first.get()));
        iv.emplace_back((double)t0, (double)t0 + ms);
        g.timed_ms += ms;
        g.timed_launches += 1;
    }
    std::sort(iv.begin(), iv.end());
    double lo = 0.0, hi = -1.0;
    for (const auto& x : iv) {
        if (hi < lo || x.first > hi) { if (hi > lo) g.timed_busy_ms += hi - lo; lo = x.first; hi = x.second; }
        else if (x.second > hi) hi = x.second;
    }
    if (hi > lo) g.timed_busy_ms += hi - lo;
    g.ev_used = 0;
    *total_ms = g.timed_ms;
    *launches = g.timed_launches;
    return RC_OK;
}
int rc_gemm_timing_busy(rc_ctx* ctx, double* busy_ms) {
    if (!ctx || !busy_ms) return RC_ERR_INVALID;
    *busy_ms = ctx->gemm->timed_busy_ms;
    return RC_OK;
}

}
```

### robustcap_amd/csrc/rc_gemm_lds.hip

```cpp
#include "rc_internal.h"
#include <hip/hip_ext.h>
#include "rc_gates.h"

typedef float f32x4 __attribute__((ext_vector_type(4)));
typedef float f32x2 __attribute__((ext_vector_type(2)));
typedef unsigned int u32x4 __attribute__((ext_vector_type(4)));
typedef unsigned int u32x2 __attribute__((ext_vector_type(2)));
typedef __bf16 bf16x8 __attribute__((ext_vector_type(8)));

#ifdef RC_TRACE_TILES
__device__ unsigned long long* g_lds_trace_buf = nullptr;
__device__ unsigned long long g_lds_trace_cap = 0;
__device__ unsigned long long g_lds_trace_n = 0;
extern "C" int rc_trace_lds_set(unsigned long long* buf, unsigned long long cap_records) {
    const unsigned long long zero = 0;
    if (hipMemcpyToSymbol(HIP_SYMBOL(g_lds_trace_buf), &buf, sizeof(buf)) != hipSuccess) return -1;
    if (hipMemcpyToSymbol(HIP_SYMBOL(g_lds_trace_n), &zero, sizeof(zero)) != hipSuccess) return -1;
    return hipMemcpyToSymbol(HIP_SYMBOL(g_lds_trace_cap), &cap_records, sizeof(cap_records)) == hipSuccess ? 0 : -1;
}
#define LDS_T(i) do { if (threadIdx.x == 0) trace_t[i] = wall_clock64(); } while (0)
#define LDS_TRACE_OUT(LAST)                                                                                                  \
    do { if (threadIdx.x == 0 && g_lds_trace_buf) {                                                                          \
        const unsigned long long idx = atomicAdd(&g_lds_trace_n, 1ull);                                                      \
        if (idx < g_lds_trace_cap) { unsigned long long* r_ = g_lds_trace_buf + idx * 8;                                     \
            r_[0] = (unsigned long long)P.H | ((unsigned long long)kh0 << 16) | ((unsigned long long)P.ksplit << 20) | ((unsigned long long)(LAST) << 24) | (1ull << 32);  \
            r_[1] = __smid(); r_[2] = trace_t[0]; r_[3] = trace_t[1]; r_[4] = trace_t[2]; r_[5] = trace_t[3]; r_[6] = wall_clock64(); r_[7] = nrows; } } } while (0)
#else
#define LDS_T(i) do { } while (0)
#define LDS_TRACE_OUT(LAST) do { } while (0)
#endif

#ifndef RC_LAND
#define RC_LAND 1
#endif

namespace {

constexpr int kWaves = 8;
constexpr int kStage = 8 * 3 * 1024;
constexpr int kRing = 4;
constexpr int kPW = 3;
constexpr int kCnt = 3 * kWaves;
constexpr int kRowIdle = (int)0x80000000u;
constexpr int kRowMask = 0x7fffffff;

#define RC_MFMA(A, B, C) C = __builtin_amdgcn_mfma_f32_16x16x32_bf16(__builtin_bit_cast(bf16x8, A), __builtin_bit_cast(bf16x8, B), C, 0, 0, 0)

__device__ __forceinline__ void split_pair(const f32x2 a, unsigned& h, unsigned& m, unsigned& l) {
    const u32x2 ua = __builtin_bit_cast(u32x2, a);
    const f32x2 r1 = a - __builtin_bit_cast(f32x2, ua & 0xffff0000u);
    const u32x2 um = __builtin_bit_cast(u32x2, r1);
    const f32x2 r2 = r1 - __builtin_bit_cast(f32x2, um & 0xffff0000u);
    const u32x2 ul = __builtin_bit_cast(u32x2, r2);
    h = __builtin_amdgcn_perm(ua[1], ua[0], 0x07060302u);
    m = __builtin_amdgcn_perm(um[1], um[0], 0x07060302u);
    l = __builtin_amdgcn_perm(ul[1], ul[0], 0x07060302u);
}
__device__ __forceinline__ void split_block(const f32x4& x0, const f32x4& x1, u32x4& h, u32x4& m, u32x4& l) {
    const f32x2 a[4] = {f32x2{x0[0], x0[1]}, f32x2{x0[2], x0[3]}, f32x2{x1[0], x1[1]}, f32x2{x1[2], x1[3]}};
#pragma unroll
    for (int d = 0; d < 4; ++d) {
        unsigned hh, mm, ll;
        split_pair(a[d], hh, mm, ll);
        h[d] = hh; m[d] = mm; l[d] = ll;
    }
}

__device__ __forceinline__ void gload(f32x4& d, const float* p) { asm volatile("global_load_dwordx4 %0, %1, off" : "=v"(d) : "v"(p) : "memory"); }
__device__ __forceinline__ void gload1k(f32x4& d, const float* p) { asm volatile("global_load_dwordx4 %0, %1, off offset:1024" : "=v"(d) : "v"(p) : "memory"); }
template <int OFF>
__device__ __forceinline__ void glds(const u32x4* g, unsigned lds_) {
    const unsigned lds = __builtin_amdgcn_readfirstlane(lds_);
    unsigned keep;
    asm volatile("s_mov_b32 %0, m0\n\ts_mov_b32 m0, %2\n\ts_nop 0\n\tglobal_load_lds_dwordx4 %1, off offset:%3\n\ts_mov_b32 m0, %0"
                 : "=&s"(keep) : "v"(g), "s"(lds), "n"(OFF) : "memory");
}
template <int OFF>
__device__ __forceinline__ void dsread(u32x4& d, unsigned addr) { asm volatile("ds_read_b128 %0, %1 offset:%2" : "=v"(d) : "v"(addr), "n"(OFF) : "memory"); }
template <int N>
__device__ __forceinline__ void wait_vm() { asm volatile("s_waitcnt vmcnt(%0)" :: "n"(N) : "memory"); }

template <int CTRL>
__device__ __forceinline__ float quad(float v) {
    return __builtin_bit_cast(float, __builtin_amdgcn_mov_dpp(__builtin_bit_cast(int, v), CTRL, 0xf, 0xf, true));
}
__device__ __forceinline__ void quad_transpose(const f32x4& v, const int q, f32x4& g) {
    const bool odd = q & 1, hi = q & 2;
    const float x0 = quad<0xB1>(v[0]), x1 = quad<0xB1>(v[1]), x2 = quad<0xB1>(v[2]), x3 = quad<0xB1>(v[3]);
    const float a0 = odd ? x1 : v[0], a1 = odd ? v[1] : x0, a2 = odd ? x3 : v[2], a3 = odd ? v[3] : x2;
    const float y0 = quad<0x4E>(a0), y1 = quad<0x4E>(a1), y2 = quad<0x4E>(a2), y3 = quad<0x4E>(a3);
    g[0] = hi ? y2 : a0; g[1] = hi ? y3 : a1; g[2] = hi ? a2 : y0; g[3] = hi ? a3 : y1;
}

template <int MAXP, typename PP>
__device__ __forceinline__ bool locate(const PP Lp, const int Ln, const int item, int& pi, int& m_tile, int& n_tile, int& kh0, int& kh1) {
    pi = 0;
#pragma unroll
    for (int q = 1; q < MAXP; ++q)
        if (q < Ln && item >= Lp[q].wg_base) pi = q;
    const auto& P = Lp[pi];
    const int local = item - P.wg_base;
    const int t = P.ksplit == 2 ? local >> 1 : local;
    kh0 = P.ksplit == 2 ? (local & 1) : 0;
    kh1 = P.ksplit == 2 ? kh0 + 1 : 2;
    n_tile = t % P.n_tiles;
    m_tile = t / P.n_tiles;
    return m_tile < P.m_tiles;
}

struct HalfArgs {
    const float* pa[2];
    const u32x4* pw;
    unsigned rd0;
    unsigned my_lds;
    int Qh, Qq;
    bool primed;
};

template <int NR, bool SHORT_OK>
__device__ __forceinline__ void k_half(const HalfArgs& c, f32x4 (&acc0)[2][8], f32x4 (&acc1)[2][8]) {
    constexpr int NA = 2 * NR;
    f32x4 raw[2][2][2];
    u32x4 pl[2][3];
    u32x4 bf[2][3];
    const int Qh = c.Qh;
#define ISSUE_A(BUF, QI)                                                                                                    \
    do {                                                                                                                    \
        const long long ko_ = (long long)min((QI), Qh - 1) * 512;                                                           \
        if constexpr (NR > 0) { gload(raw[BUF][0][0], c.pa[0] + ko_); gload1k(raw[BUF][0][1], c.pa[0] + ko_); }             \
        if constexpr (NR > 1) { gload(raw[BUF][1][0], c.pa[1] + ko_); gload1k(raw[BUF][1][1], c.pa[1] + ko_); }             \
    } while (0)
#define ISSUE_B(QI)                                                                                                         \
    do {                                                                                                                    \
        const u32x4* g_ = c.pw + (long long)min((QI), Qh - 1) * 192;                                                        \
        const unsigned dst_ = c.my_lds + (unsigned)((QI) & (kRing - 1)) * kStage;                                           \
        glds<0>(g_, dst_); glds<1024>(g_, dst_); glds<2048>(g_, dst_);                                                      \
    } while (0)
#define TIE_RAW(BUF)                                                                                                        \
    do {                                                                                                                    \
        if constexpr (NR > 0) asm volatile("" : "+v"(raw[BUF][0][0]), "+v"(raw[BUF][0][1]));                                \
        if constexpr (NR > 1) asm volatile("" : "+v"(raw[BUF][1][0]), "+v"(raw[BUF][1][1]));                                \
    } while (0)
#define SLOT(J, Q, ACC)                                                                                                     \
    do {                                                                                                                    \
        constexpr int bi_ = (J) & 1;                                                                                        \
        if ((J) == 7) {        \
            wait_vm<NA + kPW>();                                                                                            \
            asm volatile("s_waitcnt lgkmcnt(0)\n\ts_barrier" ::: "memory");                                                 \
        }                                                                                                                   \
        if constexpr (NR > 0) {                                                                                             \
            if ((J) == 7) {                                                                                                 \
                const unsigned a_ = c.rd0 + (unsigned)(((Q) + 1) & (kRing - 1)) * kStage;                                   \
                dsread<0>(bf[bi_ ^ 1][0], a_); dsread<1024>(bf[bi_ ^ 1][1], a_); dsread<2048>(bf[bi_ ^ 1][2], a_);          \
            } else {                                                                                                        \
                const unsigned a_ = c.rd0 + (unsigned)((Q) & (kRing - 1)) * kStage;                                         \
                dsread<((J) + 1) * 3072>(bf[bi_ ^ 1][0], a_); dsread<((J) + 1) * 3072 + 1024>(bf[bi_ ^ 1][1], a_);          \
                dsread<((J) + 1) * 3072 + 2048>(bf[bi_ ^ 1][2], a_);                                                        \
            }                                                                                                               \
            asm volatile("s_waitcnt lgkmcnt(3)" : "+v"(bf[bi_][0]), "+v"(bf[bi_][1]), "+v"(bf[bi_][2]) :: "memory");        \
                                                     \
            RC_MFMA(pl[0][2], bf[bi_][0], ACC[0][J]); if constexpr (NR > 1) RC_MFMA(pl[1][2], bf[bi_][0], ACC[1][J]);       \
            RC_MFMA(pl[0][0], bf[bi_][2], ACC[0][J]); if constexpr (NR > 1) RC_MFMA(pl[1][0], bf[bi_][2], ACC[1][J]);       \
            RC_MFMA(pl[0][1], bf[bi_][1], ACC[0][J]); if constexpr (NR > 1) RC_MFMA(pl[1][1], bf[bi_][1], ACC[1][J]);       \
            RC_MFMA(pl[0][1], bf[bi_][0], ACC[0][J]); if constexpr (NR > 1) RC_MFMA(pl[1][1], bf[bi_][0], ACC[1][J]);       \
            RC_MFMA(pl[0][0], bf[bi_][1], ACC[0][J]); if constexpr (NR > 1) RC_MFMA(pl[1][0], bf[bi_][1], ACC[1][J]);       \
            RC_MFMA(pl[0][0], bf[bi_][0], ACC[0][J]); if constexpr (NR > 1) RC_MFMA(pl[1][0], bf[bi_][0], ACC[1][J]);       \
            __builtin_amdgcn_sched_barrier(0);                                                                              \
        }                                                                                                                   \
    } while (0)
#define ITER(CUR, Q, ACC)                                                                                                   \
    do {                                                                                                                    \
        if constexpr (NR > 0) {                                                                                             \
            wait_vm<NA + kPW>();                                                                                            \
            TIE_RAW(CUR);                                                                                                   \
            split_block(raw[CUR][0][0], raw[CUR][0][1], pl[0][0], pl[0][1], pl[0][2]);                                      \
            asm volatile("" : "+v"(pl[0][0]), "+v"(pl[0][1]), "+v"(pl[0][2]));                                              \
        }                                                                                                                   \
        if constexpr (NR > 1) {                                                                                             \
            split_block(raw[CUR][1][0], raw[CUR][1][1], pl[1][0], pl[1][1], pl[1][2]);                                      \
            asm volatile("" : "+v"(pl[1][0]), "+v"(pl[1][1]), "+v"(pl[1][2]));                                              \
        }                                                                                                                   \
        ISSUE_A(CUR, (Q) + 2);                                                                                              \
        ISSUE_B((Q) + 2);                                                                                                   \
        SLOT(0, Q, ACC); SLOT(1, Q, ACC); SLOT(2, Q, ACC); SLOT(3, Q, ACC); SLOT(4, Q, ACC); SLOT(5, Q, ACC); SLOT(6, Q, ACC); SLOT(7, Q, ACC);   \
    } while (0)

    if (c.primed) {
        ISSUE_A(0, 0); ISSUE_A(1, 1);
        wait_vm<NA>();
    } else {
        __syncthreads();
        ISSUE_A(0, 0); ISSUE_B(0); ISSUE_A(1, 1); ISSUE_B(1);
        wait_vm<NA + kPW>();
    }
    asm volatile("s_waitcnt lgkmcnt(0)\n\ts_barrier" ::: "memory");
    if constexpr (NR > 0) { dsread<0>(bf[0][0], c.rd0); dsread<1024>(bf[0][1], c.rd0); dsread<2048>(bf[0][2], c.rd0); }
#define LAND_ALL()                                                                                                          \
    do {                                                                                                                    \
        if constexpr (SHORT_OK && RC_LAND) {                                                                                \
            asm volatile("s_waitcnt vmcnt(0)\n\ts_waitcnt lgkmcnt(0)" ::: "memory");                                        \
            TIE_RAW(0); TIE_RAW(1);                                                                                         \
            if constexpr (NR > 0) asm volatile("" : "+v"(bf[0][0]), "+v"(bf[0][1]), "+v"(bf[0][2]), "+v"(bf[1][0]), "+v"(bf[1][1]), "+v"(bf[1][2])); \
        }                                                                                                                   \
    } while (0)
    LAND_ALL();
    if (SHORT_OK && c.Qq == 1) {
        ITER(0, 0, acc0); ITER(1, 1, acc1);
    } else {
        for (int q = 0; q < c.Qq; q += 2) { ITER(0, q, acc0); ITER(1, q + 1, acc0); }
        LAND_ALL();
        for (int q = c.Qq; q < Qh; q += 2) { ITER(0, q, acc1); ITER(1, q + 1, acc1); }
    }
    asm volatile("s_waitcnt vmcnt(0)\n\ts_waitcnt lgkmcnt(0)" ::: "memory");
    TIE_RAW(0); TIE_RAW(1);
    if constexpr (NR > 0) asm volatile("" : "+v"(bf[0][0]), "+v"(bf[0][1]), "+v"(bf[0][2]), "+v"(bf[1][0]), "+v"(bf[1][1]), "+v"(bf[1][2]));
#undef LAND_ALL
#undef ITER
#undef SLOT
#undef TIE_RAW
#undef ISSUE_B
#undef ISSUE_A
}

}

template <int MAXP, bool WITH_DENSE, typename PP>
__device__ __forceinline__ int lds_item(const PP Lp, const int Ln, const int LB, const int item, unsigned char* ring, int* s_rows, int* s_cnt, int* pi_out) {
#ifdef RC_TRACE_TILES
    unsigned long long trace_t[4] = {0, 0, 0, 0};
#endif
    LDS_T(0);
    int pi, m_tile, n_tile, kh0, kh1;
    const bool in_range = locate<MAXP>(Lp, Ln, item, pi, m_tile, n_tile, kh0, kh1);
    *pi_out = pi;
    if (!in_range) return 0;
#ifdef RC_SKIP_XHALF
    if (Lp[pi].epi == RC_EPI_LSTM) {
        if (Lp[pi].ksplit == 2 && kh0 == 0) return 0;
        kh0 = 1;
    }
#endif
    const auto& P = Lp[pi];
    const int B = LB;
    const int tid = threadIdx.x, lane = tid & 63;
    const int wave = __builtin_amdgcn_readfirstlane(tid >> 6);
    const int i = lane & 15, kq = lane >> 4;
    const unsigned ring0 = (unsigned)(unsigned long long)(__attribute__((address_space(3))) unsigned char*)ring;

    const int Qs = P.Qs, Qh = Qs >> 1;
    HalfArgs hc;
    hc.Qh = Qh; hc.Qq = Qh >> 1;
    hc.rd0 = ring0 + lane * 16;
    hc.my_lds = ring0 + (unsigned)wave * 3072u;
    {
        const u32x4* g_ = reinterpret_cast<const u32x4*>(P.Ws) + ((long long)(n_tile * 8 + wave) * Qs + (long long)kh0 * Qh) * 192 + lane;
        glds<0>(g_, hc.my_lds); glds<1024>(g_, hc.my_lds); glds<2048>(g_, hc.my_lds);
        glds<0>(g_ + 192, hc.my_lds + kStage); glds<1024>(g_ + 192, hc.my_lds + kStage); glds<2048>(g_ + 192, hc.my_lds + kStage);
    }
    const int lo = m_tile * 256;
    int nrows;
    if (P.flag_bit == 0) {
        nrows = min(256, B - lo);
        if (nrows <= 0) return 0;
        if (tid < 256) s_rows[tid] = lo + min(tid, nrows - 1);
        __syncthreads();
    } else {
        int total = 0, nact = 0;
        bool blocks = false;
        const bool pick = P.block_pick != 0 && B <= 256;
        for (int base = 0; base < B && total < lo + 256; base += kWaves * 64) {
            const int r = base + tid;
            const bool f = r < B && (P.flags[r] & P.flag_bit);
            const unsigned long long bal = __ballot(f);
            if (lane == 0) {
                int cnt = __popcll(bal);
                if (pick) {
                    const unsigned lo32 = (unsigned)bal, hi32 = (unsigned)(bal >> 32);
                    const unsigned bm = ((lo32 & 0xffffu) ? 1u : 0u) | ((lo32 >> 16) ? 2u : 0u) | ((hi32 & 0xffffu) ? 4u : 0u) | ((hi32 >> 16) ? 8u : 0u);
                    cnt |= (int)(bm << 16);
                    s_cnt[kWaves + 2 * wave] = (int)lo32;
                    s_cnt[kWaves + 2 * wave + 1] = (int)hi32;
                }
                s_cnt[wave] = cnt;
            }
            __syncthreads();
            int woff = 0, sum = 0;
#pragma unroll
            for (int w = 0; w < kWaves; ++w) {
                const int cw = s_cnt[w] & 0xffff;
                woff += (w < wave) ? cw : 0;
                sum += cw;
            }
            unsigned amask = 0;
            if (pick && sum > 0) {
#pragma unroll
                for (int w = 0; w < 4; ++w) amask |= (unsigned)(s_cnt[w] >> 16) << (4 * w);
                nact = __popc(amask);
                blocks = ((nact + 3) >> 2) == ((((sum + 15) >> 4) + 3) >> 2);
            }
            if (blocks) {
                if (tid < 16 * nact) {
                    int blk = 0, seen = 0;
#pragma unroll
                    for (int j = 0; j < 16; ++j) {
                        if ((amask >> j) & 1u) { if (seen == (tid >> 4)) blk = j; ++seen; }
                    }
                    const unsigned w16 = (unsigned)s_cnt[kWaves + (blk >> 1)] >> (16 * (blk & 1));
                    s_rows[tid] = (16 * blk + (tid & 15)) | (((w16 >> (tid & 15)) & 1u) ? 0 : kRowIdle);
                }
            } else {
                const int idx = total + woff + __popcll(bal & ((1ull << lane) - 1ull));
                if (f && idx >= lo && idx < lo + 256) s_rows[idx - lo] = r;
            }
            total += sum;
            __syncthreads();
        }
        nrows = blocks ? 16 * nact : min(256, total - lo);
        if (nrows <= 0) return 0;
        if (tid < 256 && tid >= nrows) s_rows[tid] = s_rows[0];
        __syncthreads();
    }
    const int tile = m_tile * P.n_tiles + n_tile;
    const int nblk = (nrows + 15) >> 4;
    const int nr = wave + 8 < nblk ? 2 : (wave < nblk ? 1 : 0);
    const int e_r[2] = {s_rows[16 * wave + i], s_rows[16 * (wave + 8) + i]};
    const int row_r[2] = {e_r[0] & kRowMask, e_r[1] & kRowMask};
    const int row_c[2] = {min(row_r[0], B - 1), min(row_r[1], B - 1)};
    const bool need_st = (P.seg[0].par_mode | P.seg[1].par_mode) != 0;
    const int st_r[2] = {need_st ? (e_r[0] >= 0 ? P.steps[row_c[0]] + P.step_off : 1) : 0, need_st ? (e_r[1] >= 0 ? P.steps[row_c[1]] + P.step_off : 1) : 0};

    const bool dense = WITH_DENSE && P.epi != RC_EPI_LSTM;
    f32x4 acc0[2][8], acc1[2][8];
    float* const my_slab = P.slab + ((long long)tile * 2) * 32768 + ((wave * 2) * 8 * 64 + lane) * 4;

    for (int kh = kh0; kh < kh1; ++kh) {
        const auto& sg = P.seg[kh];
#pragma unroll
        for (int r = 0; r < 2; ++r) {
            const int st = st_r[r];
            const int par = sg.par_mode == RC_PAR_SRC ? ((st - 1) % RC_HBUF) : (sg.par_mode == RC_PAR_DST ? (st % RC_HBUF) : 0);
            const float* a_base = sg.base;
            if (WITH_DENSE && P.sel_bit != 0 && !(P.sel_flags[row_c[r]] & P.sel_bit)) a_base = P.alt[kh];
            hc.pa[r] = a_base + (long long)par * sg.par_stride + rc_pk(row_r[r], 4 * kq, sg.ld);
        }
        hc.pw = reinterpret_cast<const u32x4*>(P.Ws) + ((long long)(n_tile * 8 + wave) * Qs + (long long)kh * Qh) * 192 + lane;
        hc.primed = kh == kh0;
#pragma unroll
        for (int r = 0; r < 2; ++r)
#pragma unroll
            for (int j = 0; j < 8; ++j) { acc0[r][j] = f32x4{0.f, 0.f, 0.f, 0.f}; acc1[r][j] = acc0[r][j]; }
        if (kh == kh0) LDS_T(1);
        if (nr == 2) k_half<2, WITH_DENSE>(hc, acc0, acc1);
        else if (nr == 1) k_half<1, WITH_DENSE>(hc, acc0, acc1);
        else k_half<0, WITH_DENSE>(hc, acc0, acc1);
        if (dense && kh == 1) {
            asm volatile("s_waitcnt vmcnt(0)" ::: "memory");
#pragma unroll
            for (int r = 0; r < 2; ++r)
                if (r < nr) {
#pragma unroll
                    for (int j = 0; j < 8; ++j) {
                        const f32x4 o = *reinterpret_cast<const f32x4*>(my_slab + (r * 8 + j) * 256);
                        acc0[r][j] = (o + acc0[r][j]) + acc1[r][j];
                    }
                }
        } else {
#pragma unroll
            for (int r = 0; r < 2; ++r)
#pragma unroll
                for (int j = 0; j < 8; ++j) acc0[r][j] += acc1[r][j];
        }
        if (kh == 0) {
            float* s = my_slab;
#pragma unroll
            for (int r = 0; r < 2; ++r)
                if (r < nr) {
#pragma unroll
                    for (int j = 0; j < 8; ++j) *reinterpret_cast<f32x4*>(s + (r * 8 + j) * 256) = acc0[r][j];
                }
        }
    }

    LDS_T(2);
    const int q = i & 3, u = i >> 2;
    int rr_[2], r2_[2], dst_[2];
    float c_prev[2][8], bias[8];
    const bool finisher = P.ksplit != 2 || kh0 == 1;
    if (dense) {
#pragma unroll
        for (int r = 0; r < 2; ++r) {
            rr_[r] = 16 * (wave + 8 * r) + 4 * kq + q;
            const int e_ = s_rows[rr_[r] < nrows ? rr_[r] : 0];
            if (e_ < 0) rr_[r] = 256;
            r2_[r] = min(e_ & kRowMask, B - 1);
            dst_[r] = 0;
        }
#pragma unroll
        for (int j = 0; j < 8; ++j) bias[j] = P.bias[n_tile * 128 + 16 * j + i];
    } else if (finisher) {
#pragma unroll
        for (int r = 0; r < 2; ++r) {
            rr_[r] = 16 * (wave + 8 * r) + 4 * kq + q;
            const int e_ = s_rows[rr_[r] < nrows ? rr_[r] : 0];
            if (e_ < 0) rr_[r] = 256;
            r2_[r] = min(e_ & kRowMask, B - 1);
            dst_[r] = (P.steps[r2_[r]] + P.step_off) % RC_HBUF;
#pragma unroll
            for (int j = 0; j < 8; ++j) c_prev[r][j] = P.cstate[(long long)r2_[r] * P.H + n_tile * 32 + j * 4 + u];
        }
#pragma unroll
        for (int j = 0; j < 8; ++j) bias[j] = P.bias[n_tile * 128 + 16 * j + i];
    }
#ifdef RC_SKIP_XHALF
    if (false) {
#else
    if (P.ksplit == 2) {
#endif
        if (kh0 == 0) {
            asm volatile("s_waitcnt vmcnt(0)" ::: "memory");
            __syncthreads();
            if (tid == 0) {
                __builtin_amdgcn_fence(__ATOMIC_RELEASE, "agent");
                asm volatile("s_waitcnt vmcnt(0)" ::: "memory");
                __hip_atomic_store(&P.tickets[tile], 1, __ATOMIC_RELAXED, __HIP_MEMORY_SCOPE_AGENT);
            }
            LDS_T(3); LDS_TRACE_OUT(0);
            return 0;
        }
        if (tid == 0) {
            const unsigned long long t_give_up = wall_clock64() + 200000000ull;
            while (__hip_atomic_load(&P.tickets[tile], __ATOMIC_RELAXED, __HIP_MEMORY_SCOPE_AGENT) == 0) {
                __builtin_amdgcn_s_sleep(8);
                if (wall_clock64() > t_give_up) __builtin_trap();
            }
            __hip_atomic_store(&P.tickets[tile], 0, __ATOMIC_RELAXED, __HIP_MEMORY_SCOPE_AGENT);
            __builtin_amdgcn_fence(__ATOMIC_ACQUIRE, "agent");
        }
        __syncthreads();
    } else {
        asm volatile("s_waitcnt vmcnt(0)" ::: "memory");
    }
    LDS_T(3);
#pragma unroll
    for (int r = 0; r < 2; ++r) {
        if (r >= nr) continue;
        const bool ok = rr_[r] < nrows;
        if (dense) {
#pragma unroll
            for (int j = 0; j < 8; ++j) {
                f32x4 v = acc0[r][j];
                v[0] += bias[j]; v[1] += bias[j]; v[2] += bias[j]; v[3] += bias[j];
                f32x4 g;
                quad_transpose(v, q, g);
                g[0] = fmaxf(g[0], 0.0f); g[1] = fmaxf(g[1], 0.0f); g[2] = fmaxf(g[2], 0.0f); g[3] = fmaxf(g[3], 0.0f);
                if (ok) *reinterpret_cast<f32x4*>(&P.out[rc_pk(r2_[r], n_tile * 128 + 16 * j + 4 * u, P.ldo)]) = g;
            }
            continue;
        }
        f32x4 o[8];
#pragma unroll
        for (int j = 0; j < 8; ++j) o[j] = *reinterpret_cast<const f32x4*>(my_slab + (r * 8 + j) * 256);
#pragma unroll
        for (int j = 0; j < 8; ++j) {
            f32x4 v = o[j] + acc0[r][j];
            v[0] += bias[j]; v[1] += bias[j]; v[2] += bias[j]; v[3] += bias[j];
            f32x4 g;
            quad_transpose(v, q, g);
            float cn, hn;
            rc_lstm_cell(g[0], g[1], g[2], g[3], c_prev[r][j], cn, hn);
            if (ok) {
                const int unit = n_tile * 32 + j * 4 + u;
                P.cstate[(long long)r2_[r] * P.H + unit] = cn;
                P.hstate[(long long)dst_[r] * P.h_par_stride + rc_pk(r2_[r], unit, P.H)] = hn;
            }
        }
    }
    LDS_TRACE_OUT(1);
    return 1;
}

__global__ __launch_bounds__(kWaves * 64, 1) void rc_gemm_lds_kernel(const LdsLaunch L) {
    __shared__ __attribute__((aligned(1024))) unsigned char ring[kRing * kStage];
    __shared__ int s_rows[256];
    __shared__ int s_cnt[kCnt];
    int pi;
    (void)lds_item<RC_LDS_MAXP, false, const LdsProblem*>(L.p, L.n, L.B, (int)blockIdx.x, ring, s_rows, s_cnt, &pi);
}

__device__ __forceinline__ int ld_agent(const int* p) { return __hip_atomic_load(p, __ATOMIC_RELAXED, __HIP_MEMORY_SCOPE_AGENT); }

__device__ __forceinline__ void resident_wait(const ResidentArgs& R, const __attribute__((address_space(4))) ResidentTick* T, const int k, const int pi) {
    if (threadIdx.x == 0) {
        const unsigned long long give_up = wall_clock64() + R.spin_bound;
        const int prev_items = k >= 2 ? R.item_base[k - 1] - R.item_base[k - 2] : 0;
        bool ok = false;
        for (;;) {
            ok = ld_agent(R.flag_tail) >= (T->need_tail[pi] ? k : k - 1);
            if (ok && k >= 2) ok = ld_agent(R.tick_done + (k - 2)) >= prev_items;
#pragma unroll
            for (int d = 0; d < 2; ++d)
                if (ok && T->dep[pi][d] >= 0) ok = ld_agent(R.done + (long long)(k - 1) * RC_RES_MAXP + T->dep[pi][d]) >= T->dep_items[pi][d];
            if (ok || ld_agent(R.abort) != 0) break;
            if (wall_clock64() > give_up) { __hip_atomic_store(R.abort, 1, __ATOMIC_RELAXED, __HIP_MEMORY_SCOPE_AGENT); break; }
            __builtin_amdgcn_s_sleep(4);
        }
        __builtin_amdgcn_fence(__ATOMIC_ACQUIRE, "agent");
    }
    __syncthreads();
}

__global__ __launch_bounds__(kWaves * 64, 1) void rc_gemm_resident_kernel(const ResidentArgs R) {
    __shared__ __attribute__((aligned(1024))) unsigned char ring[kRing * kStage];
    __shared__ int s_rows[256];
    __shared__ int s_cnt[kCnt];
    __shared__ int s_item;
    const int total = R.item_base[R.n_ticks];
    int k = 0;
#ifdef RC_RES_PROF
    __shared__ unsigned long long s_prof[6];
    enum { p_wait = 0, p_item = 1, p_n = 2, p_rel = 3, p_grab = 4, p_t = 5 };
    if (threadIdx.x == 0) { for (int i = 0; i < 5; ++i) s_prof[i] = 0; s_prof[p_t] = wall_clock64(); }
#define RES_STAMP(ACC) do { if (threadIdx.x == 0) { const unsigned long long n_ = wall_clock64(); s_prof[ACC] += n_ - s_prof[p_t]; s_prof[p_t] = n_; } } while (0)
#else
#define RES_STAMP(ACC) do { } while (0)
#endif
    for (;;) {
        if (threadIdx.x == 0) s_item = __hip_atomic_fetch_add(R.head, 1, __ATOMIC_RELAXED, __HIP_MEMORY_SCOPE_AGENT);
        __syncthreads();
        const int g = __builtin_amdgcn_readfirstlane(s_item);
#ifdef RC_RES_PROF
        if (g >= total) {
            if (threadIdx.x == 0) {
                unsigned long long* prof = (unsigned long long*)(((unsigned long long)(R.abort + 1) + 7ull) & ~7ull);
                for (int i = 0; i < 5; ++i) atomicAdd(prof + i, s_prof[i]);
            }
            return;
        }
        RES_STAMP(p_grab);
#endif
        if (g >= total) return;
        while (g >= R.item_base[k + 1]) ++k;
        typedef const __attribute__((address_space(4))) ResidentTick* TickC;
        const TickC T = (TickC)(unsigned long long)(R.ticks + k);
        const int item = g - R.item_base[k];
        int pi = 0;
        for (int q = 1; q < T->n; ++q) if (item >= T->p[q].wg_base) pi = q;
        resident_wait(R, T, k, pi);
        RES_STAMP(p_wait);
        typedef const __attribute__((address_space(4))) LdsProblem* ProbC;
        (void)lds_item<RC_RES_MAXP, true, ProbC>(T->p, T->n, T->B, item, ring, s_rows, s_cnt, &pi);
        RES_STAMP(p_item);
#ifdef RC_RES_PROF
        if (threadIdx.x == 0) s_prof[p_n] += 1;
#endif
        asm volatile("s_waitcnt vmcnt(0)" ::: "memory");
        __syncthreads();
        if (threadIdx.x == 0) {
            __builtin_amdgcn_fence(__ATOMIC_RELEASE, "agent");
            asm volatile("s_waitcnt vmcnt(0)" ::: "memory");
            __hip_atomic_fetch_add(R.done + (long long)k * RC_RES_MAXP + pi, 1, __ATOMIC_RELAXED, __HIP_MEMORY_SCOPE_AGENT);
            __hip_atomic_fetch_add(R.tick_done + k, 1, __ATOMIC_RELAXED, __HIP_MEMORY_SCOPE_AGENT);
            asm volatile("s_waitcnt vmcnt(0)" ::: "memory");
        }
        RES_STAMP(p_rel);
    }
}

__global__ void rc_flag_set_kernel(int* flag, int value) {
    __hip_atomic_store(flag, value, __ATOMIC_RELEASE, __HIP_MEMORY_SCOPE_AGENT);
}
__global__ void rc_flag_wait_kernel(const int* counter, int target, int* abort, unsigned long long spin_bound) {
    const unsigned long long give_up = wall_clock64() + spin_bound;
    while (ld_agent(counter) < target && ld_agent(abort) == 0) {
        if (wall_clock64() > give_up) { __hip_atomic_store(abort, 1, __ATOMIC_RELAXED, __HIP_MEMORY_SCOPE_AGENT); break; }
        __builtin_amdgcn_s_sleep(8);
    }
    __builtin_amdgcn_fence(__ATOMIC_ACQUIRE, "agent");
}

void rc_launch_gemm_resident(const ResidentArgs& R, int workgroups, hipStream_t s) {
    hipLaunchKernelGGL(rc_gemm_resident_kernel, dim3(workgroups), dim3(kWaves * 64), 0, s, R);
}
void rc_launch_flag_set(int* flag, int value, hipStream_t s) { hipLaunchKernelGGL(rc_flag_set_kernel, dim3(1), dim3(1), 0, s, flag, value); }
void rc_launch_flag_wait(const int* counter, int target, int* abort, unsigned long long spin_bound, hipStream_t s) {
    hipLaunchKernelGGL(rc_flag_wait_kernel, dim3(1), dim3(1), 0, s, counter, target, abort, spin_bound);
}

void rc_launch_gemm_lds(const LdsLaunch& L, int total_wg, hipStream_t s, hipEvent_t stop) {
    const dim3 g(total_wg), b(kWaves * 64);
    if (stop) hipExtLaunchKernelGGL(rc_gemm_lds_kernel, g, b, 0, s, nullptr, stop, 0, L);
    else hipLaunchKernelGGL(rc_gemm_lds_kernel, g, b, 0, s, L);
}
```

### robustcap_amd/csrc/rc_internal.h

```cpp
#pragma once
#include <hip/hip_runtime.h>
#include <stdint.h>
#include <memory>
#include <string>
#include <type_traits>

#define RC_MT 32
#define RC_NT 64
#ifndef RC_NW
#define RC_NW 4
#endif
#define RC_KC 16
#define RC_KALIGN 128
#define RC_HBUF 3
#define RC_MAX_PROB 14

__host__ __device__ inline long long rc_pk(long long row, int k, int ld) {
    return (row >> 4) * (16ll * ld) + (long long)(k >> 4) * 256 + ((k >> 2) & 3) * 64 + (row & 15) * 4 + (k & 3);
}

enum { RC_EPI_DENSE = 0, RC_EPI_RELU = 1, RC_EPI_LSTM = 2 };
enum { RC_PAR_NONE = 0, RC_PAR_SRC = 1, RC_PAR_DST = 2 };

#define RC_ROW_VIS 1u
#define RC_ROW_PC 2u
#define RC_ROW_UPD 4u
#define RC_ROW_REACH 8u
#define RC_ROW_MASK 16u
#define RC_ROW2_TR 1u
#define RC_ROW2_M4 2u
#define RC_ROW2_M6 4u
#define RC_ROW2_FLUSH 8u
#define RC_ROW2_VALID 16u

struct GemmSeg {
    const float* base;
    long long par_stride;
    int ld;
    int K;
    int par_mode;
    int pad_;
};

struct GemmProblem {
    GemmSeg seg[2];
    const float* W;
    const void* Ws;
    const float* bias;
    float* out;
    float* hstate;
    float* cstate;
    int* steps;
    const unsigned char* flags;
    const float* alt_base;
    const unsigned char* sel_flags;
    const unsigned char* out_flags;
    long long h_par_stride;
    int ldo, N, H;
    int out_col0, out_packed;
    int sel_bit, out_bit;
    int flag_bit;
    int epi;
    int open_step;
    int n_tiles, m_tiles, wg_base, Kp;
    int nc;
    int mr;
    int trace_base;
    int nt;
    int step_off;
};

struct GemmLaunch {
    int n;
    int B;
    int split;
    int live;
    GemmProblem p[RC_MAX_PROB];
};

#define RC_TICK_PROB 24

#define RC_LDS_MAXP 12
#define RC_LDS_SLAB_FLOATS 65536
struct LdsProblem {
    GemmSeg seg[2];
    const void* Ws;
    const float* bias;
    float* hstate;
    float* cstate;
    const int* steps;
    const unsigned char* flags;
    float* slab;
    int* tickets;
    long long h_par_stride;
    int H, flag_bit, n_tiles, m_tiles, wg_base, Qs, step_off, ksplit;
    float* out;
    const float* alt[2];
    const unsigned char* sel_flags;
    int epi, ldo, sel_bit;
    int block_pick;
};
struct LdsLaunch {
    int n, B;
    LdsProblem p[RC_LDS_MAXP];
};
#define RC_RES_MAXP 20
void rc_launch_gemm_lds(const LdsLaunch& L, int total_wg, hipStream_t s, hipEvent_t stop = nullptr);

struct ResidentTick {
    int n, B;
    LdsProblem p[RC_RES_MAXP];
    int n_items;
    int dep[RC_RES_MAXP][2];
    int dep_items[RC_RES_MAXP][2];
    int need_tail[RC_RES_MAXP];
};
struct ResidentArgs {
    const ResidentTick* ticks;
    const int* item_base;
    int n_ticks;
    int* head;
    int* done;
    int* tick_done;
    const int* flag_tail;
    int* abort;
    unsigned long long spin_bound;
};
void rc_launch_gemm_resident(const ResidentArgs& R, int workgroups, hipStream_t s);
void rc_launch_flag_set(int* flag, int value, hipStream_t s);
void rc_launch_flag_wait(const int* counter, int target, int* abort, unsigned long long spin_bound, hipStream_t s);

struct BodyConst {
    int parent[24];
    int level[24];
    float bone[24][3];
    float jrest[24][3];
    float jroot[3];
    float w33[33][24];
    float v33[33][3];
    int override_joint[33];
    int nchild[24];
    int child[24][4];
};

struct FrameBuffers {
    float *x2, *x3, *x4, *x6, *x78, *x4l, *x6l, *xi;
    float *vr, *pc, *r6d, *contact;
    float *init_out;
    unsigned char* flags;
    unsigned char* flags2;
    unsigned char* pend;
    unsigned char* regime;
    double* kconf;
    float* gravity;
    float *last_pfoot, *last_tran, *floor, *j_temp;
    int *has_last, *n_floor, *first_reach, *uv_count;
    int* trace;
    float *h2, *c2;
    int* steps2;
    long long h2_par_stride, h2_layer_stride, c2_layer_stride;
    int* frame;
    int* wsteps;
};

struct WavePrep {
    const int* frame_at;
    int* steps[6];
    const float *cx4l, *cx6l;
    int first_tick;
    int t0;
};
struct WaveTail {
    int on;
    int t_last;
    float *x4l, *x6l;
    unsigned char* flags2;
    int* wsteps;
    int *steps4, *steps6;
    float *cx4l, *cx6l;
};

struct FrameIO {
    const float *j2d, *acc, *ori, *first_tran;
    float *pose_out, *tran_out;
    long long s_j2d, s_acc, s_ori, s_pose, s_tran;
    const int* len;
    int t;
};
__host__ __device__ inline bool rc_row_live(const FrameIO& io, int row, int t) { return !io.len || t < io.len[row]; }

struct rc_params_dev {
    double conf_lo, conf_hi, tran_filter_num;
    float contact_threshold, distance_threshold, height_threshold;
    int use_flat_floor, use_vision_updater, use_imu_updater, live, update_vision_freq, use_reproj_opt;
    float smooth;
};

#define RC_LIVE_MAXB 4
struct LiveGrid { int hot; int st[4][RC_LIVE_MAXB]; int act[4][RC_LIVE_MAXB]; int pre; int pre_base; const float* prebuf; };
struct LiveNet {
    const float *W1, *b1;
    const float *Wl[2], *bl[2];
    const float *W2, *b2;
    float *x1, *h, *c, *part;
    int* steps;
    int H, out, outp, Kp1;
    long long BpH;
};
struct LiveFrame {
    LiveNet net[6];
    FrameBuffers fb;
    FrameIO io;
    rc_params_dev prm;
    const BodyConst* body;
    int* status;
    int* abort;
    unsigned* spin_mb;
    unsigned* spin_state;
    LiveGrid* hot[4];
    unsigned* done_flag;
    unsigned* done_seq;
    int B;
    int nc;
};
#define RC_LIVE_KERNELS 7
struct LiveKernel {
    const void* fn;
    const char* name;
    unsigned grid;
    int has_grid;
    unsigned wg;
    LiveFrame F;
    LiveGrid G;
};
int rc_live_plan(const LiveFrame& F, LiveKernel* out, const float* prebuf = nullptr);
int rc_live_pre_plan(const LiveFrame& F, float* prebuf, LiveKernel* out);
long long rc_live_pre_floats(const LiveFrame& F);
void rc_launch_live_frame(const LiveFrame& F, hipStream_t s, const float* prebuf = nullptr);
void rc_launch_live_pre(const LiveFrame& F, float* prebuf, hipStream_t s);

struct AqlChain;
int rc_aql_create(int hip_device, AqlChain** out, char* err, int err_len);
int rc_aql_add(AqlChain* c, const LiveKernel* k, int n, int frame, char* err, int err_len);
int rc_aql_run(AqlChain* c, int prog);
int rc_aql_submit(AqlChain* c, int prog);
int rc_aql_alloc_shared(AqlChain* c, size_t bytes, void** ptr);
int rc_aql_submit_ahead(AqlChain* c, int prog, int beside);
unsigned long long rc_aql_seq(const AqlChain* c);
int rc_aql_wait_seq(AqlChain* c, unsigned long long seq);
int rc_aql_wait_frame(AqlChain* c);
int rc_aql_fence_background(AqlChain* c);
void rc_aql_set_mailbox(AqlChain* c, volatile unsigned* mb);
int rc_aql_arm(AqlChain* c);
int rc_aql_wait_background(AqlChain* c);
void rc_aql_destroy(AqlChain* c);

void rc_launch_gemm(const GemmLaunch& L, int total_wg, hipStream_t s, hipEvent_t stop = nullptr);
void rc_launch_scan_conf(const float* j2d, long long row_stride, int B, int T, double conf_lo, double conf_hi, signed char* codes, hipStream_t s,
                         float* means = nullptr, const int* len = nullptr, int len_t0 = 0);
void rc_launch_advance_steps(int* const* steps6, int n_frames, int B, hipStream_t s);
bool rc_gemm_is_w32(const GemmLaunch& L);
bool rc_gemm_is_small(const GemmLaunch& L);
void rc_launch_prep(const FrameBuffers& fb, const FrameIO& io, const rc_params_dev& prm, int B, int first_frame, hipStream_t s);
void rc_launch_fuse(const FrameBuffers& fb, const FrameIO& io, const rc_params_dev& prm, int B, hipStream_t s);
void rc_launch_tail(const FrameBuffers& fb, const FrameIO& io, const rc_params_dev& prm, const BodyConst* body, int B,
                    int first_frame, hipStream_t s, const FrameIO* io_next = nullptr,
                    const WaveTail* wt = nullptr, hipEvent_t stop = nullptr);
bool rc_launch_fuse_tail(const FrameBuffers& fb_tail, const FrameBuffers& fb_fuse, const FrameIO& io, const rc_params_dev& prm, const BodyConst* body, int B,
                         const WaveTail& wt, hipStream_t s, hipEvent_t stop);
void rc_launch_prep_wave(const FrameBuffers& slot, const FrameIO& io0, const rc_params_dev& prm, int B, const WavePrep& w, hipStream_t s);
void rc_launch_reset(const FrameBuffers& fb, float* const* h, float* const* c, const int* hidden, const unsigned char* mask,
                     int B, hipStream_t s);

void rc_launch_flush_flags(const FrameBuffers& fb, int B, hipStream_t s);
void rc_launch_pack_rows(const float* src, int src_ld, int cols, float* dst, int ld, int B, hipStream_t s);

void rc_launch_r6d(const float* r6d, float* R, long long n, hipStream_t s);
struct CamConst { float Kinv[9]; float R[9]; };
void rc_launch_camera_inputs(const float* kp, const float* acc, const float* ori, const CamConst& cam, float* j2dc, float* accc,
// ... 244 lines not shown
```

### robustcap_amd/csrc/rc_sequence_api.cpp

```cpp
#include "../../include/robustcap_hip.h"
#include "rc_ctx.h"

#include <algorithm>
#include <chrono>
#include <cstdio>
#include <cstring>
#include <initializer_list>
#include <vector>

#define RC_SPLIT_MAIN_MIN_BATCH 48

namespace {

enum { SEQ_STEPPED_TR = 0, SEQ_STEPPED = 1 };
const int kRing = 16;

enum { G_BIG = 0, G_REST = 1, G_LIN2 = 2 };
struct TickStage { int kind; int net; int stage; int group; };
const TickStage kTick[RC_TICK_PROB] = {
    {1, N4, 2, G_BIG}, {2, N4, 3, G_BIG}, {1, N6, 6, G_BIG}, {2, N6, 7, G_BIG},
    {1, N2, 2, G_REST}, {2, N2, 3, G_REST}, {1, N3, 6, G_REST}, {2, N3, 7, G_REST}, {1, N7, 6, G_REST}, {2, N7, 7, G_REST}, {1, N8, 6, G_REST}, {2, N8, 7, G_REST},
    {0, N4, 1, G_REST}, {0, N2, 1, G_REST}, {0, N6, 5, G_REST}, {0, N3, 5, G_REST}, {0, N7, 5, G_REST}, {0, N8, 5, G_REST},
    {3, N4, 4, G_LIN2}, {3, N2, 4, G_LIN2}, {3, N6, 8, G_LIN2}, {3, N3, 8, G_LIN2}, {3, N7, 8, G_LIN2}, {3, N8, 8, G_LIN2}};
const int kFuseStage = 4, kTailStage = 8, kInitStage = 5;
// ... 320 lines not shown
        const int kind = q < RC_TICK_PROB ? kTick[q].kind : 4;
        const int riders = P.n_rider[e];
        const int rows = kind == 4 ? P.n_reach[e] : ((net == N4 || net == N6) ? P.n_vis[e] + riders : P.n_valid[e]);
        if (rows <= 0) continue;
        const int rows_k = kind == 4 ? rows : rows + (rows_as_padded ? P.done(e) : 0);
        GemmProblem p = ctx->seq->wave2_prob[(size_t)(e % kRing) * W2_PROB + q];
        if (kind == 0 || kind == 1) {
            float* x1 = e % 3 == 0 ? ctx->net[net].x1 : (e % 3 == 1 ? ctx->seq->x1_alt[net] : ctx->seq->x1_alt2[net]);
            if (kind == 0) p.out = x1; else p.seg[0].base = x1;
        }
        if (kind == 1 || kind == 2) {
            const NetDev& n = ctx->net[net];
            int mr, nc;
            if (lds_problem(ctx, rows_k)) {
                mr = 16; nc = 8;
            } else if (gemm_split(ctx) && rows_k >= tile64_rows) {
                const int* t = n.H == 512 ? tiles.t5 : (n.H == 1024 ? tiles.t6 : tiles.t4);
                mr = t[0]; nc = t[1];
            } else {
                pick_tile(n.H, rows_k, &mr, &nc);
            }
            p.mr = mr; p.nc = nc; p.n_tiles = n.H / (4 * nc);
        } else if (kind == 0 || kind == 4) {
            if (rows_k <= 16) { p.mr = 1; p.nc = 1; p.n_tiles = (p.N + 15) / 16; }
            else if (kind == 0 && gemm_split(ctx) && rows_k >= tile64_rows) {
                const int np = round_up(p.N, 64);
                if (np % 128 == 0) { p.mr = 4; p.nc = 8; p.n_tiles = np / 128; }
            }
        }
        p.m_tiles = (rows + 16 * p.mr - 1) / (16 * p.mr);
        if (rows == B && kind != 4) {
            p.flags = nullptr; p.flag_bit = 0;
            if (riders == 0 && (net == N4 || net == N6) && P.n_vis[e] == B) {
                p.alt_base = nullptr; p.sel_flags = nullptr; p.sel_bit = 0; p.out_flags = nullptr; p.out_bit = 0;
            }
        }
        ps.push_back(p);
    }
    if (g != G_LIN2) {
        int total = 0;
        for (const GemmProblem& p : ps) total += p.n_tiles * p.m_tiles;
        if (total > 0 && total <= 128)
            for (GemmProblem& p : ps)
                if (p.epi == RC_EPI_LSTM && p.mr == 4 && p.nc == 8) { p.nc = 4; p.n_tiles *= 2; }
    }
    return ps;
}

struct WaveSeg {
    rc_ctx* ctx; const WavePlan& P; const FrameIO& io0; hipStream_t st, aux;
    WaveEngine eng; WaveTiles tiles; rc_params_dev prm; WavePrep wp; WaveTail wt;
    int rows(const std::vector<int>& v, int tick) const { return tick >= 0 && tick < P.n_prep ? v[tick] : 0; }
    std::vector<GemmProblem> group(int k, int g) const { return collect(ctx, P, eng, tiles, k, g); }
};

void wave_prep(WaveSeg& S, int k) {
    if (k >= S.P.n_prep) return;
    S.wp.frame_at = S.ctx->seq->frame_at_d.get() + (size_t)k * S.ctx->B;
    S.wp.first_tick = k == 0 ? 1 : 0;
    rc_launch_prep_wave(S.ctx->seq->ring2[k % kRing], S.io0, S.prm, S.ctx->B, S.wp, S.aux);
}

int wave_lin2_fuse_tail(WaveSeg& S, int k, bool merge, hipEvent_t signal) {
    rc_ctx* ctx = S.ctx;
    const int B = ctx->B;
    if (int rc = launch_problems(ctx, S.group(k, G_LIN2), nullptr, S.aux, true)) return rc;
    const bool fuse = S.rows(S.P.n_valid, k - kFuseStage) > 0, tail = S.rows(S.P.n_valid, k - kTailStage) > 0;
    bool merged = false, carried = false;
    if (tail) {
        const FrameBuffers& tgt = ctx->seq->ring2[k % kRing];
        S.wt.x4l = tgt.x4l; S.wt.x6l = tgt.x6l; S.wt.flags2 = tgt.flags2; S.wt.wsteps = tgt.wsteps;
    }
    if (merge && fuse && tail)
        merged = carried = rc_launch_fuse_tail(ctx->seq->ring2[(k - kTailStage) % kRing], ctx->seq->ring2[(k - kFuseStage) % kRing], S.io0, S.prm, ctx->body, B, S.wt, S.aux, signal);
    if (!merged && fuse) rc_launch_fuse(ctx->seq->ring2[(k - kFuseStage) % kRing], S.io0, S.prm, B, S.aux);
    if (!merged && tail) {
        rc_launch_tail(ctx->seq->ring2[(k - kTailStage) % kRing], S.io0, S.prm, ctx->body, B, 0, S.aux, nullptr, &S.wt, signal);
        carried = true;
    }
    if (signal && !carried) HIP_TRY(ctx, hipEventRecord(signal, S.aux));
    return RC_OK;
}

inline int wave_wait(rc_ctx* ctx, int k, hipStream_t s, std::initializer_list<hipEvent_t> waits) {
    if (k > 0) for (hipEvent_t w : waits) if (w) HIP_TRY(ctx, hipStreamWaitEvent(s, w, 0));
    return RC_OK;
}

int wave_issue(rc_ctx* ctx, int k, hipStream_t s, std::initializer_list<hipEvent_t> waits, const std::vector<GemmProblem>& ps, hipEvent_t signal) {
    if (int rc = wave_wait(ctx, k, s, waits)) return rc;
    bool carried = false;
    if (int rc = launch_problems(ctx, ps, nullptr, s, false, signal, &carried)) return rc;
    if (signal && !carried) HIP_TRY(ctx, hipEventRecord(signal, s));
    return RC_OK;
}

int stream_tick(WaveSeg& S, int k) {
    rc_ctx* ctx = S.ctx;
    const int e = k & 3, ep = (k + 3) & 3;
    hipStream_t st = S.st, aux = S.aux, w2 = ctx->seq->wide2_stream.get(), w3 = ctx->seq->wide3_stream.get();
    hipEvent_t main_p = ctx->seq->ev_main[ep].get(), aux_p = ctx->seq->ev_aux[ep].get(), w2_p = ctx->seq->ev_wide2[ep].get(), w3_p = ctx->seq->ev_wide3[ep].get(),
               head_p = ctx->seq->ev_head[ep].get();
    hipEvent_t main_e = ctx->seq->ev_main[e].get(), aux_e = ctx->seq->ev_aux[e].get(), w2_e = ctx->seq->ev_wide2[e].get(), w3_e = ctx->seq->ev_wide3[e].get(),
               head_e = ctx->seq->ev_head[e].get();
    bool init_now = false;
    for (int q = W2_INIT0; q < W2_PROB; ++q) init_now = init_now || S.rows(S.P.n_reach, k - w2_stage(q)) > 0;
    if (S.eng == ENG_TRI) {
        std::vector<GemmProblem> l1, rnn6, h512;
        for (const GemmProblem& p : S.group(k, G_REST)) (p.epi != RC_EPI_LSTM ? l1 : (p.H == 1024 ? rnn6 : h512)).push_back(p);
        if (int rc = wave_issue(ctx, k, aux, {}, l1, head_e)) return rc;
        wave_prep(S, k);
        if (int rc = wave_wait(ctx, k, aux, {w3_p, main_p, w2_p})) return rc;
        if (int rc = wave_lin2_fuse_tail(S, k, true, aux_e)) return rc;
        if (int rc = wave_issue(ctx, k, w2, {head_p}, rnn6, w2_e)) return rc;
        static const int h5_early = tune_env("RC_SEQ_H5_EARLY", 0);
        const bool early = h5_early && S.rows(S.P.n_reach, k - 1 - kTailStage) == 0;
        if (int rc = wave_issue(ctx, k, w3, {early ? head_p : aux_p}, h512, w3_e)) return rc;
        if (int rc = wave_issue(ctx, k, st, {head_p}, S.group(k, G_BIG), main_e)) return rc;
    } else if (S.eng == ENG_SPLIT) {
        if (int rc = wave_wait(ctx, k, aux, {main_p, w2_p})) return rc;
        wave_prep(S, k);
        if (int rc = wave_lin2_fuse_tail(S, k, false, aux_e)) return rc;
        if (int rc = wave_issue(ctx, k, w2, {aux_p}, S.group(k, G_REST), w2_e)) return rc;
        if (int rc = wave_issue(ctx, k, st, {w2_p, init_now ? aux_p : nullptr}, S.group(k, G_BIG), main_e)) return rc;
    } else {
        if (int rc = wave_wait(ctx, k, aux, {main_p})) return rc;
        wave_prep(S, k);
        if (int rc = wave_lin2_fuse_tail(S, k, false, aux_e)) return rc;
        if (int rc = wave_issue(ctx, k, st, {init_now ? aux_p : nullptr}, S.group(k, G_BIG), nullptr)) return rc;
        if (int rc = wave_issue(ctx, k, st, {init_now ? nullptr : aux_p}, S.group(k, G_REST), main_e)) return rc;
    }
    ctx->seq->stat_ticks += 1;
    return RC_OK;
}

struct ResidentWords { int *item_base, *done, *tick_done, *words; };

int build_resident_ticks(WaveSeg& S, std::vector<std::vector<GemmProblem>>& init_l) {
    rc_ctx* ctx = S.ctx;
    int run = 0;
    for (int k = 0; k < S.P.n_ticks; ++k) {
        std::vector<GemmProblem> ls;
        for (int g : {G_BIG, G_REST})
            for (GemmProblem& p : S.group(k, g)) {
                if (p.epi == RC_EPI_LSTM) { p.mr = 16; p.nc = 8; }
                else if (p.epi == RC_EPI_RELU && p.out_packed && p.N % 128 == 0 && p.Kp % 128 == 0 && p.out_bit == 0 && p.out_col0 == 0 && p.seg[0].par_mode == 0 &&
                         p.out != ctx->hid1 && p.out != ctx->hid2) { }
                else { init_l[k].push_back(p); continue; }
                p.m_tiles = 1;
                ls.push_back(p);
            }
        ResidentTick& T = ctx->seq->res_ticks_h[k];
        LdsRegion region{};
        if (int rc = lds_region(ctx, (size_t)(k & 3), &region)) return rc;
        size_t tiles = 0;
        T.B = ctx->B;
        T.n = build_lds_problems(ctx, ls, nullptr, region.slab, region.tickets, T.p, RC_RES_MAXP, &T.n_items, &tiles, true);
        if (T.n != (int)ls.size()) return fail(ctx, RC_ERR_INVALID, "resident engine: more problems in a tick than its table holds");
        if (tiles > region.tiles) return fail(ctx, RC_ERR_INVALID, "resident engine: more tiles in a tick than a slab region holds");
        const bool tail_wrote = S.rows(S.P.n_reach, k - 1 - kTailStage) > 0;
        for (int i = 0; i < RC_RES_MAXP; ++i) {
            T.dep[i][0] = T.dep[i][1] = -1; T.dep_items[i][0] = T.dep_items[i][1] = 0;
            T.need_tail[i] = 0;
            if (i >= T.n) continue;
            const bool lstm = T.p[i].epi == RC_EPI_LSTM;
            T.need_tail[i] = lstm ? ((tail_wrote && T.p[i].H == 512) ? 1 : 0) : 1;
            if (k == 0 || !lstm) continue;
            const ResidentTick& Tp = ctx->seq->res_ticks_h[k - 1];
            for (int j = 0; j < Tp.n; ++j) {
                const int items_j = (j + 1 < Tp.n ? Tp.p[j + 1].wg_base : Tp.n_items) - Tp.p[j].wg_base;
                const bool lstm_j = Tp.p[j].epi == RC_EPI_LSTM;
                if (lstm_j && Tp.p[j].hstate == T.p[i].hstate) { T.dep[i][0] = j; T.dep_items[i][0] = items_j; }
                if ((const float*)(lstm_j ? Tp.p[j].hstate : Tp.p[j].out) == T.p[i].seg[0].base) { T.dep[i][1] = j; T.dep_items[i][1] = items_j; }
            }
        }
        ctx->seq->res_base_h[k] = run;
        run += T.n_items;
    }
    ctx->seq->res_base_h[S.P.n_ticks] = run;
    return RC_OK;
}

int run_resident_segment(WaveSeg& S) {
    rc_ctx* ctx = S.ctx;
    hipStream_t st = S.st, aux = S.aux;
    const int res_wgs = std::min(240, std::max(8, ctx->seq->resident_wgs));
    LdsRegion pool{};
    if (int rc = lds_region(ctx, 0, &pool)) return rc;
    if (!ctx->seq->res_abort_h) {
        HIP_TRY(ctx, rc_alloc(ctx->seq->res_abort_h, 1));
        ctx->seq->res_abort_h[0] = 0;
    }
    const size_t nt = (size_t)S.P.n_ticks;
    if (nt > ctx->seq->res_cap) {
        HIP_TRY(ctx, hipDeviceSynchronize());
        const size_t cap = nt + nt / 4 + 64;
        HIP_TRY(ctx, rc_grow(ctx->seq->res_cap, nt, cap, ctx->seq->res_ticks_d, cap, ctx->seq->res_ticks_h, cap,
                             ctx->seq->res_ints_d, cap * (RC_RES_MAXP + 2) + 1 + 4 + 16, ctx->seq->res_base_h, cap + 1));
    }
    const size_t cap = ctx->seq->res_cap;
    ResidentWords W{};
    W.item_base = ctx->seq->res_ints_d.get(); W.done = W.item_base + cap + 1; W.tick_done = W.done + cap * RC_RES_MAXP; W.words = W.tick_done + cap;
    std::vector<std::vector<GemmProblem>> init_l(nt);
    if (int rc = build_resident_ticks(S, init_l)) return rc;
    HIP_TRY(ctx, hipMemcpyAsync(ctx->seq->res_ticks_d.get(), ctx->seq->res_ticks_h.get(), nt * sizeof(ResidentTick), hipMemcpyHostToDevice, st));
    HIP_TRY(ctx, hipMemcpyAsync(W.item_base, ctx->seq->res_base_h.get(), (nt + 1) * sizeof(int), hipMemcpyHostToDevice, st));
    HIP_TRY(ctx, hipMemsetAsync(W.done, 0, (cap * (RC_RES_MAXP + 1) + 4 + 16) * sizeof(int), st));
    HIP_TRY(ctx, hipEventRecord(ctx->seq->ev_main[6].get(), st));
    HIP_TRY(ctx, hipStreamWaitEvent(aux, ctx->seq->ev_main[6].get(), 0));
    ResidentArgs R{};
    R.ticks = ctx->seq->res_ticks_d.get(); R.item_base = W.item_base; R.n_ticks = S.P.n_ticks;
    R.head = W.words; R.done = W.done; R.tick_done = W.tick_done;
    R.flag_tail = W.words + 2; R.abort = W.words + 3;
    R.spin_bound = (unsigned long long)std::max(1, tune_env("RC_SEQ_RESIDENT_BOUND_MS", 2000)) * 100000ull;
    if (int rc = timed_launch(ctx, st, LAUNCH_RESIDENT, [&] { rc_launch_gemm_resident(R, res_wgs, st); })) return rc;
    count_resident_launch(ctx);
    for (int k = 0; k < S.P.n_ticks; ++k) {
        if (int rc = launch_problems(ctx, init_l[k], nullptr, aux, false)) return rc;
        wave_prep(S, k);
        if (k > 0) rc_launch_flag_wait(W.tick_done + (k - 1), ctx->seq->res_ticks_h[k - 1].n_items, W.words + 3, R.spin_bound, aux);
        if (int rc = wave_lin2_fuse_tail(S, k, false, nullptr)) return rc;
        rc_launch_flag_set(W.words + 2, k + 1, aux);
        ctx->seq->stat_ticks += 1;
    }
    HIP_TRY(ctx, hipEventRecord(ctx->seq->ev_aux[0].get(), aux));
    HIP_TRY(ctx, hipStreamWaitEvent(st, ctx->seq->ev_aux[0].get(), 0));
    HIP_TRY(ctx, hipMemcpyAsync(ctx->seq->res_abort_h.get(), W.words + 3, sizeof(int), hipMemcpyDeviceToHost, st));
    HIP_TRY(ctx, hipGetLastError());
#ifdef RC_RES_PROF
    {
        HIP_TRY(ctx, hipStreamSynchronize(st));
        unsigned long long ph[5];
        const unsigned long long* pd = (const unsigned long long*)(((unsigned long long)(W.words + 4) + 7ull) & ~7ull);
        if (hipMemcpy(ph, pd, sizeof(ph), hipMemcpyDeviceToHost) == hipSuccess && ph[2] > 0)
            std::fprintf(stderr, "[res prof] %d ticks, %llu items on %d workgroups; per item: wait %.2f us, item %.2f us, release %.2f us, take %.2f us; per workgroup %.2f ms\n",
                         S.P.n_ticks, ph[2], res_wgs, ph[0] / 100.0 / ph[2], ph[1] / 100.0 / ph[2], ph[3] / 100.0 / ph[2], ph[4] / 100.0 / ph[2],
                         (ph[0] + ph[1] + ph[3] + ph[4]) / 100.0 / 1000.0 / res_wgs);
    }
#endif
    ctx->seq->stat_resident_segments += 1;
    return RC_OK;
}

int run_wave2_segment(rc_ctx* ctx, const WavePlan& P, const FrameIO& io0, int t0, int t_last, hipStream_t st) {
    const int B = ctx->B;
    const size_t need = (size_t)P.n_prep * B;
    if (need > ctx->seq->frame_at_cap) {
        HIP_TRY(ctx, hipDeviceSynchronize());
        if (int rc = reserve_frame_at(ctx, need, need + need / 4 + 4096)) return rc;
    }
    std::memcpy(ctx->seq->frame_at_h.get(), P.frame_at.data(), need * sizeof(int));
    HIP_TRY(ctx, hipMemcpyAsync(ctx->seq->frame_at_d.get(), ctx->seq->frame_at_h.get(), need * sizeof(int), hipMemcpyHostToDevice, st));

    const WaveEngine eng = pick_wave_engine(ctx);
    WaveSeg S{ctx, P, io0, st, ctx->seq->aux_stream.get(), eng, wave_tiles(eng), dev_params(ctx->prm), WavePrep{}, WaveTail{}};
    for (int i = 0; i < 6; ++i) S.wp.steps[i] = ctx->net[i].steps;
    S.wp.cx4l = ctx->fb.x4l; S.wp.cx6l = ctx->fb.x6l; S.wp.t0 = t0;
    S.wt.on = 1; S.wt.t_last = t_last;
    S.wt.steps4 = ctx->net[N4].steps; S.wt.steps6 = ctx->net[N6].steps;
    S.wt.cx4l = ctx->fb.x4l; S.wt.cx6l = ctx->fb.x6l;
    hipStream_t w2 = ctx->seq->wide2_stream.get(), w3 = ctx->seq->wide3_stream.get();
    HIP_TRY(ctx, hipEventRecord(ctx->seq->ev_main[7].get(), st));
    HIP_TRY(ctx, hipStreamWaitEvent(S.aux, ctx->seq->ev_main[7].get(), 0));
    if (eng != ENG_PLAIN) HIP_TRY(ctx, hipStreamWaitEvent(w2, ctx->seq->ev_main[7].get(), 0));
    if (eng == ENG_TRI) HIP_TRY(ctx, hipStreamWaitEvent(w3, ctx->seq->ev_main[7].get(), 0));
    if (resident_segment(ctx, eng, P)) {
        if (int rc = run_resident_segment(S)) return rc;
    } else {
        for (int k = 0; k < P.n_ticks; ++k) if (int rc = stream_tick(S, k)) return rc;
        const int last = (P.n_ticks - 1) & 3;
        if (P.n_ticks > 0) {
            HIP_TRY(ctx, hipStreamWaitEvent(st, ctx->seq->ev_aux[last].get(), 0));
            if (eng != ENG_PLAIN) HIP_TRY(ctx, hipStreamWaitEvent(st, ctx->seq->ev_wide2[last].get(), 0));
            if (eng == ENG_TRI) {
                HIP_TRY(ctx, hipStreamWaitEvent(st, ctx->seq->ev_head[last].get(), 0));
                HIP_TRY(ctx, hipStreamWaitEvent(st, ctx->seq->ev_wide3[last].get(), 0));
                HIP_TRY(ctx, hipStreamWaitEvent(st, ctx->seq->ev_main[last].get(), 0));
            }
        }
        HIP_TRY(ctx, hipGetLastError());
    }
    ctx->seq->stat_wave_frames += t_last - t0 + 1;
    return RC_OK;
}

int reserve_plan_tables(rc_ctx* ctx, int T) {
    const size_t B = (size_t)ctx->B;
    const size_t need = B * (size_t)T;
    HIP_TRY(ctx, rc_grow(ctx->seq->scan_cap, need, need, ctx->seq->scan_codes_d, need, ctx->seq->scan_codes_h, need));
    if (!ctx->seq->scan_state_h) HIP_TRY(ctx, rc_alloc(ctx->seq->scan_state_h, B * 3));
    const size_t fneed = B * ((size_t)T + 64);
    return reserve_frame_at(ctx, fneed, fneed);
}

}

int seq_prepare(rc_ctx* ctx) {
    if (!ctx->seq->seq_mode || ctx->prm.live) return RC_OK;
    if (int rc = ensure_wave2_buffers(ctx)) return rc;
    if (int rc = build_wave2_problems(ctx)) return rc;
    return reserve_plan_tables(ctx, 1024);
}

extern "C" {

static int sequence_impl(rc_ctx* ctx, int32_t T, const int32_t* len, int32_t off, const float* j2dc, int64_t rs_j2d, const float* accc,
                         int64_t rs_acc, const float* oric, int64_t rs_ori, const float* first_tran, uint32_t flags, float* pose_out,
                         int64_t rs_pose, float* tran_out, int64_t rs_tran, void* stream) {
    std::vector<int> rows_len;
    if (len) {
        rows_len.resize(ctx->B);
        int longest = 0;
        bool same = true;
        for (int b = 0; b < ctx->B; ++b) {
            rows_len[b] = std::max(0, std::min(len[b] - off, T));
            longest = std::max(longest, rows_len[b]);
            same = same && rows_len[b] == rows_len[0];
        }
        if (longest == 0) return RC_OK;
        T = longest;
        if (same) rows_len.clear();
    }
    const int* L = rows_len.empty() ? nullptr : rows_len.data();
    const int* len_d = L ? ctx->seq->row_len_d.get() : nullptr;
    const int32_t kMaxPlanFrames = std::max(8, tune_env("RC_SEQ_MAX_PLAN_FRAMES", 4096));
    if (T > kMaxPlanFrames && ctx->seq->seq_mode && !ctx->prm.live) {
        for (int32_t a = 0; a < T; a += kMaxPlanFrames) {
            const int32_t n = std::min(kMaxPlanFrames, T - a);
            if (int rc = sequence_impl(ctx, n, L ? len : nullptr, off + a, j2dc + (int64_t)a * 99, rs_j2d, accc + (int64_t)a * 18, rs_acc, oric + (int64_t)a * 54, rs_ori,
                                     a == 0 ? first_tran : nullptr, a == 0 ? flags : 0u, pose_out + (int64_t)a * 216, rs_pose,
                                     tran_out + (int64_t)a * 3, rs_tran, stream)) return rc;
        }
        return RC_OK;
    }
    hipStream_t st = (hipStream_t)stream;
    auto io_at = [&](int t) {
        return FrameIO{j2dc + (int64_t)t * 99, accc + (int64_t)t * 18, oric + (int64_t)t * 54, t == 0 ? first_tran : nullptr,
                       pose_out + (int64_t)t * 216, tran_out + (int64_t)t * 3, rs_j2d, rs_acc, rs_ori, rs_pose, rs_tran, len_d, off + t};
    };
    std::vector<int> n_live;
    if (L) {
        n_live.assign((size_t)T + 1, 0);
        for (int b = 0; b < ctx->B; ++b) n_live[L[b]] += 1;
        for (int t = T - 1, run = n_live[T]; t >= 0; --t) { const int ends = n_live[t]; n_live[t] = run; run += ends; }
        n_live.resize(T);
    }
    {
        long long rf = 0;
        if (L) for (int b = 0; b < ctx->B; ++b) rf += L[b]; else rf = (long long)ctx->B * T;
        ctx->seq->stat_row_frames += rf;
    }
    std::vector<unsigned char> mode((size_t)(T > 0 ? T : 0), (unsigned char)SEQ_STEPPED_TR);
    const int B = ctx->B;
    WavePlan wplan;
    int wave2_from = -1;
    const int w0 = ((flags & RC_FLAG_FIRST_FRAME) || first_tran) ? 1 : 0;
    if (ctx->seq->seq_mode && !ctx->prm.live && T >= 2 && T - w0 >= std::max(1, ctx->seq->seq_min_frames)) {
        if (int rc = ensure_wave2_buffers(ctx)) return rc;
        if (!ctx->seq->wave2_valid) if (int rc = build_wave2_problems(ctx)) return rc;
        const size_t need = (size_t)B * T;
        if (need > ctx->seq->scan_cap || !ctx->seq->scan_state_h) {
            HIP_TRY(ctx, hipStreamSynchronize(st));
            if (int rc = reserve_plan_tables(ctx, T)) return rc;
        }
        rc_launch_scan_conf(j2dc, rs_j2d, B, T, ctx->prm.conf_lo, ctx->prm.conf_hi, ctx->seq->scan_codes_d.get(), st, nullptr, len_d, off);
        HIP_TRY(ctx, hipMemcpyAsync(ctx->seq->scan_codes_h.get(), ctx->seq->scan_codes_d.get(), need, hipMemcpyDeviceToHost, st));
        HIP_TRY(ctx, hipMemcpyAsync(ctx->seq->scan_state_h.get(), ctx->fb.first_reach, (size_t)B * sizeof(int), hipMemcpyDeviceToHost, st));
// ... 170 lines not shown
```

### robustcap_amd/net/sig_mp.py

```python
import ctypes as C
import os

import numpy as np
import torch

from .. import _lib
from .. import body as _body
from .. import config as cfg

_PARAM_ATTRS = {"use_flat_floor", "use_vision_updater", "use_imu_updater", "live", "conf_range", "tran_filter_num",
                "contact_threshold", "distrance_threshold", "height_threhold", "update_vision_freq", "use_reproj_opt",
                "smooth"}


class _ModuleView:

    def __init__(self, net, prefix):
        self.__dict__["_net"], self.__dict__["_prefix"] = net, prefix

    def _keys(self):
        return [k for k, _ in cfg.state_dict_spec() if k.startswith(self._prefix + ".")]

    def __getattr__(self, name):
        full = self._prefix + "." + name
# ... 324 lines not shown
                pose, tran = torch.empty(24, 3, 3), torch.empty(3)
                rc = self._lib.rc_live_step(self._ctx, j2dc.data_ptr(), accc.data_ptr(), oric.data_ptr(), None,
                                            _lib.RC_FLAG_FIRST_FRAME if first_frame else 0, pose.data_ptr(), tran.data_ptr())
                if rc:
                    _lib.check(self._ctx, rc, "rc_live_step")
                return pose, tran
            p, t = self.forward_live(j2dc, accc, oric, first_tran, first_frame)
            return p[0], t[0]
        pose, tran = self.forward_batch(j2dc, accc, oric, first_tran, first_frame)
        return pose[0].cpu(), tran[0].cpu()

    @torch.no_grad()
    def forward_live(self, j2dc, accc, oric, first_tran=None, first_frame=False):
        B = self.batch
        self._sync_gravity()
        if not self.__dict__.get("_live_on"):
            torch.cuda.synchronize()
            _lib.check(self._ctx, self._lib.rc_live_begin(self._ctx), "rc_live_begin")
            self.__dict__["_live_on"] = True
        def host(x, n):
            if isinstance(x, torch.Tensor) and x.dtype == torch.float32 and x.device.type == "cpu" and x.is_contiguous() and x.numel() == n:
                return x
            return torch.as_tensor(x, dtype=torch.float32).cpu().reshape(n).contiguous()
        j2dc, accc, oric = host(j2dc, B * 99), host(accc, B * 18), host(oric, B * 54)
        ft = None if first_tran is None else host(first_tran, B * 3)
        pose, tran = torch.empty(B, 24, 3, 3), torch.empty(B, 3)
        rc = self._lib.rc_live_step(self._ctx, j2dc.data_ptr(), accc.data_ptr(), oric.data_ptr(), None if ft is None else ft.data_ptr(),
                                    _lib.RC_FLAG_FIRST_FRAME if first_frame else 0, pose.data_ptr(), tran.data_ptr())
        _lib.check(self._ctx, rc, "rc_live_step")
        return pose, tran

    def fusion_state(self):
        t = torch.empty(self.batch, 5, dtype=torch.int32)
        _lib.check(self._ctx, self._lib.rc_get_fusion_state(self._ctx, _lib.ptr(t), _lib.stream_ptr()), "rc_get_fusion_state")
        return t

    def live_stats(self):
        a, b = C.c_int64(0), C.c_int64(0)
        _lib.check(self._ctx, self._lib.rc_get_live_stats(self._ctx, C.byref(a), C.byref(b)), "rc_get_live_stats")
        return a.value, b.value

    def live_prestep_stats(self):
        a, b = C.c_int64(0), C.c_int32(0)
        _lib.check(self._ctx, self._lib.rc_get_live_prestep(self._ctx, C.byref(a), C.byref(b)), "rc_get_live_prestep")
        return a.value, bool(b.value)

    def live_spin_stats(self):
        a, b = C.c_int64(0), C.c_int64(0)
        _lib.check(self._ctx, self._lib.rc_get_live_spin(self._ctx, C.byref(a), C.byref(b)), "rc_get_live_spin")
        return a.value, b.value

    def live_replayed(self):
        a = C.c_int64(0)
        _lib.check(self._ctx, self._lib.rc_get_live_replayed(self._ctx, C.byref(a)), "rc_get_live_replayed")
        return a.value

    @torch.no_grad()
    def forward_sequence(self, j2dc, accc, oric, first_tran=None, first_frame=False, lengths=None):
        B = self.batch
        T = j2dc.shape[1]
        if lengths is not None:
            lens = np.ascontiguousarray(torch.as_tensor(lengths).detach().cpu().numpy().astype(np.int64).reshape(-1))
            if lens.shape[0] != B or (lens < 0).any() or (lens > T).any():
                raise ValueError(f"lengths: {B} values in 0 .. {T} expected")
            lens = np.ascontiguousarray(lens.astype(np.int32))
        if T == 0:
            return torch.empty(B, 0, 24, 3, 3, device=self.device), torch.empty(B, 0, 3, device=self.device)
        self._sync_gravity()
        (j2dc, rs_j), (accc, rs_a), (oric, rs_o) = self._prep_rows(j2dc, B, T, 99), self._prep_rows(accc, B, T, 18), self._prep_rows(oric, B, T, 54)
        ft = None if first_tran is None else self._prep(first_tran, (B, 3))
        pose = torch.empty(B, T, 24, 3, 3, device=self.device)
        tran = torch.empty(B, T, 3, device=self.device)
        flags = _lib.RC_FLAG_FIRST_FRAME if first_frame else 0
        if lengths is None:
            rc = self._lib.rc_sequence(self._ctx, T, _lib.ptr(j2dc), rs_j, _lib.ptr(accc), rs_a, _lib.ptr(oric), rs_o, _lib.ptr(ft),
                                       flags, _lib.ptr(pose), T * 216, _lib.ptr(tran), T * 3, _lib.stream_ptr())
            _lib.check(self._ctx, rc, "rc_sequence")
        else:
            rc = self._lib.rc_sequence_rows(self._ctx, T, lens.ctypes.data_as(C.c_void_p), _lib.ptr(j2dc), rs_j, _lib.ptr(accc), rs_a,
                                            _lib.ptr(oric), rs_o, _lib.ptr(ft), flags, _lib.ptr(pose), T * 216, _lib.ptr(tran), T * 3,
                                            _lib.stream_ptr())
            _lib.check(self._ctx, rc, "rc_sequence_rows")
        self.__dict__["_keep"] = (j2dc, accc, oric, ft)
        return pose, tran

    def sequence_row_frames(self):
        n = C.c_int64()
        _lib.check(self._ctx, self._lib.rc_get_sequence_row_frames(self._ctx, C.byref(n)), "rc_get_sequence_row_frames")
        return n.value

    @staticmethod
    def default_gemm_mode(total_rows):
        return bool(_lib.load().rc_default_gemm_mode(int(total_rows)))

    def set_gemm_mode(self, split):
        _lib.check(self._ctx, self._lib.rc_set_gemm_mode(self._ctx, int(bool(split))), "rc_set_gemm_mode")
        self.__dict__["_live_on"] = False

    @property
    def gemm_mode(self):
        return int(self._lib.rc_get_gemm_mode(self._ctx))

    def set_sequence_mode(self, enabled=True, min_frames=8, force=False):
        mode = 0 if not enabled else (2 if force else 1)
        _lib.check(self._ctx, self._lib.rc_set_sequence_mode(self._ctx, mode, int(min_frames)), "rc_set_sequence_mode")

    def sequence_stats(self):
        a, b, c = C.c_int64(), C.c_int64(), C.c_int64()
        _lib.check(self._ctx, self._lib.rc_get_sequence_stats(self._ctx, C.byref(a), C.byref(b), C.byref(c)), "rc_get_sequence_stats")
        return a.value, b.value, c.value

    def lstm_step(self, net, x, rows=None):
        spec = {n: (i, h, o) for n, i, h, o in cfg.NETS}[net]
        x = self._prep(x, (self.batch, spec[0]))
        m = None if rows is None else torch.as_tensor(rows).to(device=self.device, dtype=torch.uint8).contiguous()
        y = torch.zeros(self.batch, spec[2], device=self.device)
        _lib.check(self._ctx, self._lib.rc_lstm_step(self._ctx, net.encode(), _lib.ptr(x), _lib.ptr(m), _lib.ptr(y), _lib.stream_ptr()), "rc_lstm_step")
        torch.cuda.current_stream().synchronize()
        return y

    def get_state(self, net):
        H = {n: h for n, _, h, _ in cfg.NETS}[net]
        h = torch.empty(2, self.batch, H)
        c = torch.empty(2, self.batch, H)
        _lib.check(self._ctx, self._lib.rc_get_state(self._ctx, net.encode(), _lib.ptr(h), _lib.ptr(c), _lib.stream_ptr()), "rc_get_state")
        return h, c

    def get_trace(self):
        t = torch.empty(self.batch, 8, dtype=torch.int32)
        _lib.check(self._ctx, self._lib.rc_get_trace(self._ctx, _lib.ptr(t), _lib.stream_ptr()), "rc_get_trace")
        return t

    def gemm_kernel_name(self):
        try:
            lds, other = self.launch_stats()
        except AttributeError:
            lds, other = 0, 0
        if lds > 0:
            return "rc_gemm_lds_kernel"
        try:
            w = C.c_int64()
            _lib.check(self._ctx, self._lib.rc_get_launch_stats_w32(self._ctx, C.byref(w)), "rc_get_launch_stats_w32")
            if w.value > 0:
                return "rc_gemm_split48_w32_kernel"
        except AttributeError:
            pass
        return "rc_gemm_split_kernel" if self.gemm_mode else "rc_gemm_kernel"

    def launch_stats(self):
        a, b = C.c_int64(), C.c_int64()
        _lib.check(self._ctx, self._lib.rc_get_launch_stats(self._ctx, C.byref(a), C.byref(b)), "rc_get_launch_stats")
        return a.value, b.value

    def set_resident(self, enable=True, workgroups=0):
        _lib.check(self._ctx, self._lib.rc_set_resident(self._ctx, 1 if enable else 0, int(workgroups)), "rc_set_resident")

    def resident_stats(self):
        a, b = C.c_int64(), C.c_int64()
        _lib.check(self._ctx, self._lib.rc_get_resident_stats(self._ctx, C.byref(a), C.byref(b)), "rc_get_resident_stats")
        return a.value, b.value

    def gemm_timing(self, enable):
        _lib.check(self._ctx, self._lib.rc_gemm_timing(self._ctx, int(enable)), "rc_gemm_timing")

    def gemm_timing_read(self):
        ms, n = C.c_double(), C.c_int64()
        _lib.check(self._ctx, self._lib.rc_gemm_timing_read(self._ctx, C.byref(ms), C.byref(n)), "rc_gemm_timing_read")
        return ms.value, n.value

    def gemm_timing_busy(self):
        ms = C.c_double()
        _lib.check(self._ctx, self._lib.rc_gemm_timing_busy(self._ctx, C.byref(ms)), "rc_gemm_timing_busy")
        return ms.value

    def __del__(self):
        ctx = self.__dict__.get("_ctx")
        if ctx:
            self._lib.rc_destroy(ctx)
            self.__dict__["_ctx"] = None
```

Measured before the change: 1.282 million body-frames/s.

## Shrink LDS-GEMM split-K slab pool, split resident regions, add optional NT weight loads

Halves the per-tile split-K slab size, sizes launch and resident slab regions separately, and keeps resident ticks in their own four-region pool. The aim is a smaller scratch footprint that stays in cache. The pool is now allocated up front at weight-finalize time instead of lazily on first use. Also adds non-temporal variants of the weight-to-LDS loads behind an env flag, off by default, plus a query API for the pool. The fixed tile counts risk overflow if problem shapes exceed the assumed tile budget; the self-test only checks this for the resident path.

```diff
diff --git a/include/robustcap_hip.h b/include/robustcap_hip.h
--- a/include/robustcap_hip.h
+++ b/include/robustcap_hip.h
@@ -71,6 +71,7 @@
 int rc_get_sequence_stats(rc_ctx* ctx, int64_t* wave_frames, int64_t* stepped_frames, int64_t* ticks);
 int rc_get_launch_stats(rc_ctx* ctx, int64_t* lds_launches, int64_t* other_wide_launches);
 int rc_get_launch_stats_w32(rc_ctx* ctx, int64_t* w32_launches);
+int rc_get_lds_pool(rc_ctx* ctx, int64_t* slab_bytes, int32_t* regions, int32_t* weight_nt);
 int rc_set_resident(rc_ctx* ctx, int32_t enable, int32_t workgroups);
 int rc_get_resident_stats(rc_ctx* ctx, int64_t* segments, int64_t* aborts);
 int rc_plan_sequence(const int8_t* codes, int32_t B, int32_t T, const int32_t* pend, uint32_t flags, int32_t use_vision_updater,
diff --git a/robustcap_amd/_lib.py b/robustcap_amd/_lib.py
--- a/robustcap_amd/_lib.py
+++ b/robustcap_amd/_lib.py
@@ -54,6 +54,7 @@
     "rc_get_sequence_stats": (_I32, [_P, C.POINTER(_I64), C.POINTER(_I64), C.POINTER(_I64)]),
     "rc_get_launch_stats": (_I32, [_P, C.POINTER(_I64), C.POINTER(_I64)]),
     "rc_get_launch_stats_w32": (_I32, [_P, C.POINTER(_I64)]),
+    "rc_get_lds_pool": (_I32, [_P, C.POINTER(_I64), C.POINTER(_I32), C.POINTER(_I32)]),
     "rc_set_resident": (_I32, [_P, _I32, _I32]),
     "rc_get_resident_stats": (_I32, [_P, C.POINTER(_I64), C.POINTER(_I64)]),
     "rc_plan_sequence": (_I32, [_P, _I32, _I32, _P, _U32, _I32, _P]),
@@ -128,7 +129,7 @@
 _lib = None
 
 
-OPTIONAL_IN_AB_BUILDS = frozenset({"rc_get_launch_stats_w32", "rc_set_resident", "rc_get_resident_stats", "rc_get_launch_stats", "rc_get_live_spin", "rc_get_live_replayed", "rc_get_live_profile", "rc_get_live_last_profile",
+OPTIONAL_IN_AB_BUILDS = frozenset({"rc_get_launch_stats_w32", "rc_get_lds_pool", "rc_set_resident", "rc_get_resident_stats", "rc_get_launch_stats", "rc_get_live_spin", "rc_get_live_replayed", "rc_get_live_profile", "rc_get_live_last_profile",
                                    "rc_get_live_prestep"})
 
 
diff --git a/robustcap_amd/csrc/rc_api.cpp b/robustcap_amd/csrc/rc_api.cpp
--- a/robustcap_amd/csrc/rc_api.cpp
+++ b/robustcap_amd/csrc/rc_api.cpp
@@ -561,7 +561,8 @@
     ctx->have_weights = true;
     const bool aw = ctx->alloc_weights;
     ctx->alloc_weights = false;
-    const int rc_pre = seq_prepare(ctx);
+    int rc_pre = seq_prepare(ctx);
+    if (!rc_pre) rc_pre = gemm_prepare(ctx);
     ctx->alloc_weights = aw;
     if (rc_pre) return rc_pre;
     HIP_TRY(ctx, hipDeviceSynchronize());
diff --git a/robustcap_amd/csrc/rc_ctx.h b/robustcap_amd/csrc/rc_ctx.h
--- a/robustcap_amd/csrc/rc_ctx.h
+++ b/robustcap_amd/csrc/rc_ctx.h
@@ -111,8 +111,11 @@
 bool gemm_split(const rc_ctx* c);
 bool lds_context(const rc_ctx* c);
 bool lds_problem(const rc_ctx* c, int rows);
+bool lds_weight_nt(const rc_ctx* c);
+int gemm_prepare(rc_ctx* ctx);
 struct LdsRegion { float* slab; int* tickets; size_t tiles; };
 int lds_region(rc_ctx* ctx, size_t r, LdsRegion* out);
+int lds_resident_region(rc_ctx* ctx, size_t r, LdsRegion* out);
 int build_lds_problems(rc_ctx* ctx, const std::vector<GemmProblem>& ps, const unsigned char* flags_override, float* slab, int* tickets,
                        LdsProblem* out, int max_p, int* items, size_t* tiles_out, bool resident_order = false);
 int launch_problems(rc_ctx* ctx, std::vector<GemmProblem> ps, const unsigned char* flags_override, hipStream_t st, bool fp32 = false,
diff --git a/robustcap_amd/csrc/rc_gemm_api.cpp b/robustcap_amd/csrc/rc_gemm_api.cpp
--- a/robustcap_amd/csrc/rc_gemm_api.cpp
+++ b/robustcap_amd/csrc/rc_gemm_api.cpp
@@ -15,7 +15,9 @@
 #define RC_NC1280 10
 #endif
 
-const int kLdsRegions = 12;
+const int kLdsRegions = 10;
+const int kLdsResidentRegions = 4;
+const int kLdsLaunchTiles = 2 * (32 + 40), kLdsResidentTiles = 2 * (40 + 32 + 4 * 16) + 34;
 
 #pragma GCC visibility push(hidden)
 
@@ -39,9 +41,11 @@
     int lds_min_batch = 65;
     int lds_ksplit[3] = {1, 2, 2};
     bool lds_block_pick = true;
+    bool lds_weight_nt = false;
     DevBuf<float> lds_slab;
     DevBuf<int> lds_tickets;
     size_t lds_region_tiles = 0;
+    size_t lds_resident_tiles = 0;
     unsigned lds_rot = 0;
 };
 
@@ -58,6 +62,7 @@
     g.lds_min_rows = tune_env("RC_LDS_MIN_ROWS", std::min(160, std::max(64, batch / 2)));
     g.lds_min_batch = tune_env("RC_LDS_MIN_BATCH", g.lds_min_batch);
     g.lds_block_pick = tune_env("RC_LDS_BLOCK_PICK", 1) != 0;
+    g.lds_weight_nt = tune_env("RC_LDS_WEIGHT_NT", 0) != 0;
     g.lds_ksplit[0] = tune_env("RC_LDS_KSPLIT_512", 1) == 1 ? 1 : 2;
     g.lds_ksplit[1] = tune_env("RC_LDS_KSPLIT_1024", batch <= 160 ? 1 : 2) == 1 ? 1 : 2;
     g.lds_ksplit[2] = tune_env("RC_LDS_KSPLIT_1280", 2) == 1 ? 1 : 2;
@@ -74,6 +79,7 @@
 bool gemm_split(const rc_ctx* c) { return c->gemm->split; }
 bool lds_context(const rc_ctx* c) { return c->gemm->split && c->gemm->lds_min_rows > 0 && c->B >= c->gemm->lds_min_batch; }
 bool lds_problem(const rc_ctx* c, int rows) { return lds_context(c) && rows >= c->gemm->lds_min_rows; }
+bool lds_weight_nt(const rc_ctx* c) { return c->gemm->lds_weight_nt; }
 
 LiveLaunchScope::LiveLaunchScope(rc_ctx* c) : ctx(c) { ctx->gemm->live_launch = true; }
 LiveLaunchScope::~LiveLaunchScope() { ctx->gemm->live_launch = false; }
@@ -167,26 +173,38 @@
     return p;
 }
 
+static size_t lds_pool_tiles(const rc_ctx* ctx, size_t* region_tiles, size_t* resident_tiles) {
+    const bool replicate = std::getenv("RC_DBG_REPLICATE") != nullptr;
+    *region_tiles = (size_t)(replicate ? 320 : kLdsLaunchTiles) * (((size_t)ctx->B + 255) / 256);
+    *resident_tiles = ctx->B <= 256 ? (size_t)kLdsResidentTiles : 0;
+    return std::max((size_t)kLdsRegions * *region_tiles, (size_t)kLdsResidentRegions * *resident_tiles);
+}
 static int ensure_lds_pool(rc_ctx* ctx) {
     GemmLauncher& g = *ctx->gemm;
     if (g.lds_slab) return RC_OK;
-    const size_t m_tiles = ((size_t)ctx->B + 255) / 256;
-    const size_t tiles = 320 * m_tiles;
-    HIP_TRY(ctx, rc_alloc(g.lds_slab, (size_t)kLdsRegions * tiles * RC_LDS_SLAB_FLOATS));
-    HIP_TRY(ctx, rc_alloc(g.lds_tickets, (size_t)kLdsRegions * tiles));
-    HIP_TRY(ctx, hipMemset(g.lds_tickets.get(), 0, (size_t)kLdsRegions * tiles * sizeof(int)));
-    g.lds_region_tiles = tiles;
-    return RC_OK;
-}
-
-int lds_region(rc_ctx* ctx, size_t r, LdsRegion* out) {
+    size_t region_tiles = 0, resident_tiles = 0;
+    const size_t tiles = lds_pool_tiles(ctx, &region_tiles, &resident_tiles);
+    HIP_TRY(ctx, rc_alloc(g.lds_slab, tiles * RC_LDS_SLAB_FLOATS));
+    HIP_TRY(ctx, rc_alloc(g.lds_tickets, tiles));
+    HIP_TRY(ctx, hipMemset(g.lds_tickets.get(), 0, tiles * sizeof(int)));
+    g.lds_region_tiles = region_tiles;
+    g.lds_resident_tiles = resident_tiles;
+    return RC_OK;
+}
+int gemm_prepare(rc_ctx* ctx) { return lds_context(ctx) ? ensure_lds_pool(ctx) : RC_OK; }
+
+static int pool_region(rc_ctx* ctx, size_t r, size_t count, size_t GemmLauncher::*per_region, LdsRegion* out) {
     if (int rc = ensure_lds_pool(ctx)) return rc;
     const GemmLauncher& g = *ctx->gemm;
-    out->slab = g.lds_slab.get() + r * g.lds_region_tiles * RC_LDS_SLAB_FLOATS;
-    out->tickets = g.lds_tickets.get() + r * g.lds_region_tiles;
-    out->tiles = g.lds_region_tiles;
-    return RC_OK;
-}
+    const size_t tiles = g.*per_region;
+    if (r >= count || tiles == 0) return fail(ctx, RC_ERR_INVALID, "shared-weight kernel: no such slab region");
+    out->slab = g.lds_slab.get() + r * tiles * RC_LDS_SLAB_FLOATS;
+    out->tickets = g.lds_tickets.get() + r * tiles;
+    out->tiles = tiles;
+    return RC_OK;
+}
+int lds_region(rc_ctx* ctx, size_t r, LdsRegion* out) { return pool_region(ctx, r, kLdsRegions, &GemmLauncher::lds_region_tiles, out); }
+int lds_resident_region(rc_ctx* ctx, size_t r, LdsRegion* out) { return pool_region(ctx, r, kLdsResidentRegions, &GemmLauncher::lds_resident_tiles, out); }
 
 static bool timing_pair(GemmLauncher& g, hipEvent_t* a, hipEvent_t* b) {
     if (g.ev_used == g.ev_pool.size()) {
@@ -263,6 +281,7 @@
                              LdsLaunch& L, int* items, size_t* tiles_out) {
     L = LdsLaunch{};
     L.B = ctx->B;
+    L.weight_nt = ctx->gemm->lds_weight_nt ? 1 : 0;
     L.n = build_lds_problems(ctx, ps, flags_override, region.slab, region.tickets, L.p, RC_LDS_MAXP, items, tiles_out);
 }
 
@@ -314,7 +333,7 @@
 }
 static int dense_items_selftest(rc_ctx* ctx, const std::vector<GemmProblem>& ps, const unsigned char* flags_override, hipStream_t st) {
     LdsRegion region{};
-    if (int rc = lds_region(ctx, 0, &region)) return rc;
+    if (int rc = lds_resident_region(ctx, 0, &region)) return rc;
     const int n_ints = 2 + RC_RES_MAXP + 1 + 4;
     DevBuf<ResidentTick> tk_d;
     DevBuf<int> ints_d;
@@ -325,6 +344,7 @@
     size_t tiles = 0;
     T.B = ctx->B;
     T.n = build_lds_problems(ctx, q, flags_override, region.slab, region.tickets, T.p, RC_RES_MAXP, &T.n_items, &tiles, true);
+    if (tiles > region.tiles) return fail(ctx, RC_ERR_INVALID, "dense self-test: more tiles than a slab region holds");
     for (int i = 0; i < RC_RES_MAXP; ++i) T.dep[i][0] = T.dep[i][1] = -1;
     const int base[2] = {0, T.n_items};
     const size_t Bp = (size_t)ctx->Bp;
@@ -337,6 +357,7 @@
     R.ticks = tk_d.get(); R.item_base = ints_d.get(); R.n_ticks = 1;
     R.done = ints_d.get() + 2; R.tick_done = ints_d.get() + 2 + RC_RES_MAXP; R.head = ints_d.get() + 3 + RC_RES_MAXP; R.flag_tail = R.head + 1; R.abort = R.head + 2;
     R.spin_bound = 100000ull * 100;
+    R.weight_nt = ctx->gemm->lds_weight_nt ? 1 : 0;
     rc_launch_gemm_resident(R, 64, st);
     HIP_TRY(ctx, hipStreamSynchronize(st));
     std::vector<std::vector<float>> got(ps.size());
@@ -427,6 +448,16 @@
     return RC_OK;
 }
 
+int rc_get_lds_pool(rc_ctx* ctx, int64_t* slab_bytes, int32_t* regions, int32_t* weight_nt) {
+    if (!ctx) return RC_ERR_INVALID;
+    size_t region_tiles = 0, resident_tiles = 0;
+    const size_t tiles = lds_pool_tiles(ctx, &region_tiles, &resident_tiles);
+    if (slab_bytes) *slab_bytes = (int64_t)(tiles * RC_LDS_SLAB_FLOATS * sizeof(float));
+    if (regions) *regions = kLdsRegions;
+    if (weight_nt) *weight_nt = ctx->gemm->lds_weight_nt ? 1 : 0;
+    return RC_OK;
+}
+
 int rc_get_launch_stats(rc_ctx* ctx, int64_t* tick_launches, int64_t* other_wide_launches) {
     if (!ctx) return RC_ERR_INVALID;
     if (tick_launches) *tick_launches = ctx->gemm->stat_lds_launches;
diff --git a/robustcap_amd/csrc/rc_gemm_lds.hip b/robustcap_amd/csrc/rc_gemm_lds.hip
--- a/robustcap_amd/csrc/rc_gemm_lds.hip
+++ b/robustcap_amd/csrc/rc_gemm_lds.hip
@@ -68,12 +68,16 @@
 
 __device__ __forceinline__ void gload(f32x4& d, const float* p) { asm volatile("global_load_dwordx4 %0, %1, off" : "=v"(d) : "v"(p) : "memory"); }
 __device__ __forceinline__ void gload1k(f32x4& d, const float* p) { asm volatile("global_load_dwordx4 %0, %1, off offset:1024" : "=v"(d) : "v"(p) : "memory"); }
-template <int OFF>
+template <int OFF, bool NT>
 __device__ __forceinline__ void glds(const u32x4* g, unsigned lds_) {
     const unsigned lds = __builtin_amdgcn_readfirstlane(lds_);
     unsigned keep;
-    asm volatile("s_mov_b32 %0, m0\n\ts_mov_b32 m0, %2\n\ts_nop 0\n\tglobal_load_lds_dwordx4 %1, off offset:%3\n\ts_mov_b32 m0, %0"
-                 : "=&s"(keep) : "v"(g), "s"(lds), "n"(OFF) : "memory");
+    if constexpr (NT)
+        asm volatile("s_mov_b32 %0, m0\n\ts_mov_b32 m0, %2\n\ts_nop 0\n\tglobal_load_lds_dwordx4 %1, off offset:%3 nt\n\ts_mov_b32 m0, %0"
+                     : "=&s"(keep) : "v"(g), "s"(lds), "n"(OFF) : "memory");
+    else
+        asm volatile("s_mov_b32 %0, m0\n\ts_mov_b32 m0, %2\n\ts_nop 0\n\tglobal_load_lds_dwordx4 %1, off offset:%3\n\ts_mov_b32 m0, %0"
+                     : "=&s"(keep) : "v"(g), "s"(lds), "n"(OFF) : "memory");
 }
 template <int OFF>
 __device__ __forceinline__ void dsread(u32x4& d, unsigned addr) { asm volatile("ds_read_b128 %0, %1 offset:%2" : "=v"(d) : "v"(addr), "n"(OFF) : "memory"); }
@@ -117,7 +121,7 @@
     bool primed;
 };
 
-template <int NR, bool SHORT_OK>
+template <int NR, bool SHORT_OK, bool NT>
 __device__ __forceinline__ void k_half(const HalfArgs& c, f32x4 (&acc0)[2][8], f32x4 (&acc1)[2][8]) {
     constexpr int NA = 2 * NR;
     f32x4 raw[2][2][2];
@@ -134,7 +138,7 @@
     do {                                                                                                                    \
         const u32x4* g_ = c.pw + (long long)min((QI), Qh - 1) * 192;                                                        \
         const unsigned dst_ = c.my_lds + (unsigned)((QI) & (kRing - 1)) * kStage;                                           \
-        glds<0>(g_, dst_); glds<1024>(g_, dst_); glds<2048>(g_, dst_);                                                      \
+        glds<0, NT>(g_, dst_); glds<1024, NT>(g_, dst_); glds<2048, NT>(g_, dst_);                                                      \
     } while (0)
 #define TIE_RAW(BUF)                                                                                                        \
     do {                                                                                                                    \
@@ -224,7 +228,7 @@
 
 }
 
-template <int MAXP, bool WITH_DENSE, typename PP>
+template <int MAXP, bool WITH_DENSE, bool NT, typename PP>
 __device__ __forceinline__ int lds_item(const PP Lp, const int Ln, const int LB, const int item, unsigned char* ring, int* s_rows, int* s_cnt, int* pi_out) {
 #ifdef RC_TRACE_TILES
     unsigned long long trace_t[4] = {0, 0, 0, 0};
@@ -254,8 +258,8 @@
     hc.my_lds = ring0 + (unsigned)wave * 3072u;
     {
         const u32x4* g_ = reinterpret_cast<const u32x4*>(P.Ws) + ((long long)(n_tile * 8 + wave) * Qs + (long long)kh0 * Qh) * 192 + lane;
-        glds<0>(g_, hc.my_lds); glds<1024>(g_, hc.my_lds); glds<2048>(g_, hc.my_lds);
-        glds<0>(g_ + 192, hc.my_lds + kStage); glds<1024>(g_ + 192, hc.my_lds + kStage); glds<2048>(g_ + 192, hc.my_lds + kStage);
+        glds<0, NT>(g_, hc.my_lds); glds<1024, NT>(g_, hc.my_lds); glds<2048, NT>(g_, hc.my_lds);
+        glds<0, NT>(g_ + 192, hc.my_lds + kStage); glds<1024, NT>(g_ + 192, hc.my_lds + kStage); glds<2048, NT>(g_ + 192, hc.my_lds + kStage);
     }
     const int lo = m_tile * 256;
     int nrows;
@@ -331,7 +335,7 @@
 
     const bool dense = WITH_DENSE && P.epi != RC_EPI_LSTM;
     f32x4 acc0[2][8], acc1[2][8];
-    float* const my_slab = P.slab + ((long long)tile * 2) * 32768 + ((wave * 2) * 8 * 64 + lane) * 4;
+    float* const my_slab = P.slab + (long long)tile * RC_LDS_SLAB_FLOATS + ((wave * 2) * 8 * 64 + lane) * 4;
 
     for (int kh = kh0; kh < kh1; ++kh) {
         const auto& sg = P.seg[kh];
@@ -350,9 +354,9 @@
 #pragma unroll
             for (int j = 0; j < 8; ++j) { acc0[r][j] = f32x4{0.f, 0.f, 0.f, 0.f}; acc1[r][j] = acc0[r][j]; }
         if (kh == kh0) LDS_T(1);
-        if (nr == 2) k_half<2, WITH_DENSE>(hc, acc0, acc1);
-        else if (nr == 1) k_half<1, WITH_DENSE>(hc, acc0, acc1);
-        else k_half<0, WITH_DENSE>(hc, acc0, acc1);
+        if (nr == 2) k_half<2, WITH_DENSE, NT>(hc, acc0, acc1);
+        else if (nr == 1) k_half<1, WITH_DENSE, NT>(hc, acc0, acc1);
+        else k_half<0, WITH_DENSE, NT>(hc, acc0, acc1);
         if (dense && kh == 1) {
             asm volatile("s_waitcnt vmcnt(0)" ::: "memory");
 #pragma unroll
@@ -479,13 +483,16 @@
     return 1;
 }
 
-__global__ __launch_bounds__(kWaves * 64, 1) void rc_gemm_lds_kernel(const LdsLaunch L) {
+template <bool NT>
+__device__ __forceinline__ void lds_launch_body(const LdsLaunch& L) {
     __shared__ __attribute__((aligned(1024))) unsigned char ring[kRing * kStage];
     __shared__ int s_rows[256];
     __shared__ int s_cnt[kCnt];
     int pi;
-    (void)lds_item<RC_LDS_MAXP, false, const LdsProblem*>(L.p, L.n, L.B, (int)blockIdx.x, ring, s_rows, s_cnt, &pi);
-}
+    (void)lds_item<RC_LDS_MAXP, false, NT, const LdsProblem*>(L.p, L.n, L.B, (int)blockIdx.x, ring, s_rows, s_cnt, &pi);
+}
+__global__ __launch_bounds__(kWaves * 64, 1) void rc_gemm_lds_kernel(const LdsLaunch L) { lds_launch_body<false>(L); }
+__global__ __launch_bounds__(kWaves * 64, 1) void rc_gemm_lds_nt_kernel(const LdsLaunch L) { lds_launch_body<true>(L); }
 
 __device__ __forceinline__ int ld_agent(const int* p) { return __hip_atomic_load(p, __ATOMIC_RELAXED, __HIP_MEMORY_SCOPE_AGENT); }
 
@@ -509,7 +516,8 @@
     __syncthreads();
 }
 
-__global__ __launch_bounds__(kWaves * 64, 1) void rc_gemm_resident_kernel(const ResidentArgs R) {
+template <bool NT>
+__device__ __forceinline__ void resident_body(const ResidentArgs& R) {
     __shared__ __attribute__((aligned(1024))) unsigned char ring[kRing * kStage];
     __shared__ int s_rows[256];
     __shared__ int s_cnt[kCnt];
@@ -548,7 +556,7 @@
         resident_wait(R, T, k, pi);
         RES_STAMP(p_wait);
         typedef const __attribute__((address_space(4))) LdsProblem* ProbC;
-        (void)lds_item<RC_RES_MAXP, true, ProbC>(T->p, T->n, T->B, item, ring, s_rows, s_cnt, &pi);
+        (void)lds_item<RC_RES_MAXP, true, NT, ProbC>(T->p, T->n, T->B, item, ring, s_rows, s_cnt, &pi);
         RES_STAMP(p_item);
 #ifdef RC_RES_PROF
         if (threadIdx.x == 0) s_prof[p_n] += 1;
@@ -565,6 +573,8 @@
         RES_STAMP(p_rel);
     }
 }
+__global__ __launch_bounds__(kWaves * 64, 1) void rc_gemm_resident_kernel(const ResidentArgs R) { resident_body<false>(R); }
+__global__ __launch_bounds__(kWaves * 64, 1) void rc_gemm_resident_nt_kernel(const ResidentArgs R) { resident_body<true>(R); }
 
 __global__ void rc_flag_set_kernel(int* flag, int value) {
     __hip_atomic_store(flag, value, __ATOMIC_RELEASE, __HIP_MEMORY_SCOPE_AGENT);
@@ -579,7 +589,7 @@
 }
 
 void rc_launch_gemm_resident(const ResidentArgs& R, int workgroups, hipStream_t s) {
-    hipLaunchKernelGGL(rc_gemm_resident_kernel, dim3(workgroups), dim3(kWaves * 64), 0, s, R);
+    hipLaunchKernelGGL(R.weight_nt ? rc_gemm_resident_nt_kernel : rc_gemm_resident_kernel, dim3(workgroups), dim3(kWaves * 64), 0, s, R);
 }
 void rc_launch_flag_set(int* flag, int value, hipStream_t s) { hipLaunchKernelGGL(rc_flag_set_kernel, dim3(1), dim3(1), 0, s, flag, value); }
 void rc_launch_flag_wait(const int* counter, int target, int* abort, unsigned long long spin_bound, hipStream_t s) {
@@ -588,6 +598,7 @@
 
 void rc_launch_gemm_lds(const LdsLaunch& L, int total_wg, hipStream_t s, hipEvent_t stop) {
     const dim3 g(total_wg), b(kWaves * 64);
-    if (stop) hipExtLaunchKernelGGL(rc_gemm_lds_kernel, g, b, 0, s, nullptr, stop, 0, L);
-    else hipLaunchKernelGGL(rc_gemm_lds_kernel, g, b, 0, s, L);
-}
+    const auto kernel = L.weight_nt ? rc_gemm_lds_nt_kernel : rc_gemm_lds_kernel;
+    if (stop) hipExtLaunchKernelGGL(kernel, g, b, 0, s, nullptr, stop, 0, L);
+    else hipLaunchKernelGGL(kernel, g, b, 0, s, L);
+}
diff --git a/robustcap_amd/csrc/rc_internal.h b/robustcap_amd/csrc/rc_internal.h
--- a/robustcap_amd/csrc/rc_internal.h
+++ b/robustcap_amd/csrc/rc_internal.h
@@ -81,7 +81,7 @@
 #define RC_TICK_PROB 24
 
 #define RC_LDS_MAXP 12
-#define RC_LDS_SLAB_FLOATS 65536
+#define RC_LDS_SLAB_FLOATS 32768
 struct LdsProblem {
     GemmSeg seg[2];
     const void* Ws;
@@ -102,6 +102,7 @@
 };
 struct LdsLaunch {
     int n, B;
+    int weight_nt;
     LdsProblem p[RC_LDS_MAXP];
 };
 #define RC_RES_MAXP 20
@@ -125,6 +126,7 @@
     const int* flag_tail;
     int* abort;
     unsigned long long spin_bound;
+    int weight_nt;
 };
 void rc_launch_gemm_resident(const ResidentArgs& R, int workgroups, hipStream_t s);
 void rc_launch_flag_set(int* flag, int value, hipStream_t s);
diff --git a/robustcap_amd/csrc/rc_sequence_api.cpp b/robustcap_amd/csrc/rc_sequence_api.cpp
--- a/robustcap_amd/csrc/rc_sequence_api.cpp
+++ b/robustcap_amd/csrc/rc_sequence_api.cpp
@@ -496,7 +496,7 @@
             }
         ResidentTick& T = ctx->seq->res_ticks_h[k];
         LdsRegion region{};
-        if (int rc = lds_region(ctx, (size_t)(k & 3), &region)) return rc;
+        if (int rc = lds_resident_region(ctx, (size_t)(k & 3), &region)) return rc;
         size_t tiles = 0;
         T.B = ctx->B;
         T.n = build_lds_problems(ctx, ls, nullptr, region.slab, region.tickets, T.p, RC_RES_MAXP, &T.n_items, &tiles, true);
@@ -530,7 +530,7 @@
     hipStream_t st = S.st, aux = S.aux;
     const int res_wgs = std::min(240, std::max(8, ctx->seq->resident_wgs));
     LdsRegion pool{};
-    if (int rc = lds_region(ctx, 0, &pool)) return rc;
+    if (int rc = lds_resident_region(ctx, 0, &pool)) return rc;
     if (!ctx->seq->res_abort_h) {
         HIP_TRY(ctx, rc_alloc(ctx->seq->res_abort_h, 1));
         ctx->seq->res_abort_h[0] = 0;
@@ -557,6 +557,7 @@
     R.head = W.words; R.done = W.done; R.tick_done = W.tick_done;
     R.flag_tail = W.words + 2; R.abort = W.words + 3;
     R.spin_bound = (unsigned long long)std::max(1, tune_env("RC_SEQ_RESIDENT_BOUND_MS", 2000)) * 100000ull;
+    R.weight_nt = lds_weight_nt(ctx) ? 1 : 0;
     if (int rc = timed_launch(ctx, st, LAUNCH_RESIDENT, [&] { rc_launch_gemm_resident(R, res_wgs, st); })) return rc;
     count_resident_launch(ctx);
     for (int k = 0; k < S.P.n_ticks; ++k) {
diff --git a/robustcap_amd/net/sig_mp.py b/robustcap_amd/net/sig_mp.py
--- a/robustcap_amd/net/sig_mp.py
+++ b/robustcap_amd/net/sig_mp.py
@@ -500,6 +500,11 @@
         _lib.check(self._ctx, self._lib.rc_get_launch_stats(self._ctx, C.byref(a), C.byref(b)), "rc_get_launch_stats")
         return a.value, b.value
 
+    def lds_pool(self):
+        b, r, nt = C.c_int64(), C.c_int32(), C.c_int32()
+        _lib.check(self._ctx, self._lib.rc_get_lds_pool(self._ctx, C.byref(b), C.byref(r), C.byref(nt)), "rc_get_lds_pool")
+        return b.value, r.value, bool(nt.value)
+
     def set_resident(self, enable=True, workgroups=0):
         _lib.check(self._ctx, self._lib.rc_set_resident(self._ctx, 1 if enable else 0, int(workgroups)), "rc_set_resident")
 
```

After: 1.280 million body-frames/s. About the same (-0.2%).
